# fr34kcoders/storb

Hardware: AMD Instinct MI355X
Metric: GiB/s device-resident RS encode+decode, 1 MiB chunks, 1/2/4/8 MI355X (higher is better)
Workload: dtype u8; 1 GPU; 1024 x 1 MiB chunks per GPU, RS(k=4,m=2)=zfec(4,6): encode + decode/reassemble with data shards {1,3} erased; chunks_per_gpu=1024, chunk_bytes=1048576, k=4, m_total=6, world_size=1, parallelism=chunk-partition x1

## Files before the change

include/storb_ec.h:

```cpp
#ifndef STORB_EC_H
#define STORB_EC_H

#include <stddef.h>
#include <stdint.h>

#ifdef __cplusplus
extern "C" {
#endif

#define SEC_ABI_VERSION 1

enum sec_status {
    SEC_OK = 0,
    SEC_EINVAL = -1,
    SEC_EKM = -2,
    SEC_EBLOCKLEN = -3,
    SEC_ENBLOCKS = -4,
    SEC_ESHARENUM = -5,
    SEC_EDUPSHARE = -6,
    SEC_EPADLEN = -7,
    SEC_ESIZE = -8,
    SEC_ENODEV = -9,
    SEC_EHIP = -10,
    SEC_ENOMEM = -11,
// ... 134 lines not shown
                           const int32_t *target_nums, const uint64_t *target_offs, uint8_t *out,
                           uint8_t *digests, sec_chk_result *results, uint8_t *row_bad,
                           uint8_t *column, unsigned flags);

int sec_check_locate(int k, int m, const int32_t *sharenums, int n, const uint8_t *column,
                     int32_t *culprit);

int sec_check_method(int k, int m, const int32_t *sharenums, int n, uint64_t B,
                     const uint64_t *block_avail, int64_t padlen, int *method);

int sec_ctx_check_methods(sec_ctx *ctx, int64_t *bitsliced, int64_t *direct);

int sec_repair_method(int k, int m, const int32_t *sharenums, int n, const int32_t *targets,
                      int ntargets, uint64_t B, const uint64_t *block_avail, int *method);

int sec_ctx_repair_methods(sec_ctx *ctx, int64_t *bitsliced, int64_t *direct);

typedef struct sec_msg {
    uint64_t addr;
    uint64_t len;
    uint64_t avail;
} sec_msg;

int sec_sha1_batch(sec_ctx *ctx, const sec_msg *msgs, int64_t nmsgs, uint8_t *digests, unsigned flags);

int sec_encode_digest_batch(sec_ctx *ctx, const sec_enc_chunk *chunks, int64_t nchunks,
                            const uint8_t *in, uint8_t *parity, uint8_t *digests, unsigned flags);

int sec_encode_pieces(sec_ctx *ctx, const sec_enc_chunk *chunks, int64_t nchunks, const uint8_t *in,
                      uint8_t *const *pieces, uint8_t *digests, unsigned flags);

typedef struct sec_bn_key sec_bn_key;

int sec_bn_key_create(sec_ctx *ctx, const uint8_t n_be[256], sec_bn_key **out);
void sec_bn_key_destroy(sec_bn_key *key);
int sec_bn_key_set_crt(sec_ctx *ctx, sec_bn_key *key, const uint8_t p_be[128], const uint8_t q_be[128],
                       const uint8_t cp_be[256], const uint8_t cq_be[256]);
int sec_bn_key_set_tag(sec_ctx *ctx, sec_bn_key *key, const uint8_t g_be[256], const uint8_t fdh_be[256],
                       const uint8_t d_be[256], const uint8_t *dp_be, const uint8_t *dq_be);

int sec_bn_reduce_batch(sec_ctx *ctx, const sec_bn_key *key, const sec_msg *msgs, int64_t nmsgs,
                        uint8_t *out, unsigned flags);
int sec_bn_modexp_batch(sec_ctx *ctx, const sec_bn_key *key, const uint8_t *bases,
                        const uint8_t *exps, uint32_t exp_bytes, int64_t count, uint8_t *out,
                        unsigned flags);
int sec_bn_crt_modexp_batch(sec_ctx *ctx, const sec_bn_key *key, const uint8_t *bases,
                            const uint8_t *exps_p, const uint8_t *exps_q, uint32_t exp_bytes,
                            int64_t count, uint8_t *out, unsigned flags);
int sec_apdp_gpow_batch(sec_ctx *ctx, const sec_bn_key *key, const uint8_t *exps, uint32_t exp_bytes,
                        int64_t count, uint8_t *out, unsigned flags);
int sec_bn_mulmod_batch(sec_ctx *ctx, const sec_bn_key *key, const uint8_t *a, const uint8_t *b,
                        int64_t count, uint8_t *out, unsigned flags);
int sec_apdp_tag_batch(sec_ctx *ctx, const sec_bn_key *key, const sec_msg *msgs, int64_t nmsgs,
                       uint8_t *tags, unsigned flags);

int sec_bn_crt_modexp2_batch(sec_ctx *ctx, const sec_bn_key *key, const uint8_t *a, const uint8_t *b,
                             const uint8_t *ea_p, const uint8_t *ea_q, const uint8_t *eb_p,
                             const uint8_t *eb_q, uint32_t exp_bytes, int64_t count, uint8_t *out,
                             unsigned flags);
int sec_apdp_prove_batch(sec_ctx *ctx, const sec_bn_key *key, const sec_msg *msgs, int64_t nmsgs,
                         const uint8_t *tags, const uint8_t *g_ss, const uint8_t *coefs,
                         uint8_t *tag_c, uint8_t *block, uint8_t *rho, unsigned flags);
int sec_apdp_verify_batch(sec_ctx *ctx, const sec_bn_key *key, const uint8_t *proof_tags,
                          const uint8_t *fdhs, const uint8_t *coefs, const uint8_t *ss,
                          const uint8_t e_be[256], int64_t count, uint8_t *values, int32_t *status,
                          unsigned flags);

int sec_encode_tag_batch(sec_ctx *ctx, const sec_bn_key *key, const sec_enc_chunk *chunks,
                         int64_t nchunks, const uint8_t *in, uint8_t *parity,
                         uint8_t *digests , uint8_t *tags, unsigned flags);
int sec_encode_pieces_tags(sec_ctx *ctx, const sec_bn_key *key, const sec_enc_chunk *chunks,
                           int64_t nchunks, const uint8_t *in, uint8_t *const *pieces,
                           uint8_t *digests , uint8_t *tags, unsigned flags);

int sec_malloc(sec_ctx *ctx, size_t bytes, void **dptr);
int sec_free(sec_ctx *ctx, void *dptr);
int sec_host_alloc(sec_ctx *ctx, size_t bytes, void **hptr);
int sec_host_free(sec_ctx *ctx, void *hptr);
int sec_host_register(sec_ctx *ctx, void *hptr, size_t bytes);
int sec_host_unregister(sec_ctx *ctx, void *hptr);
int sec_ctx_host_paths(sec_ctx *ctx, int64_t *zero_copy, int64_t *registered, int64_t *staged);
int sec_host_pinned_bytes(int64_t *loaned, int64_t *idle);
int sec_ctx_decode_paths(sec_ctx *ctx, int64_t *syndrome, int64_t *direct);
int sec_ctx_decode_methods(sec_ctx *ctx, int64_t *fused, int64_t *pair, int64_t *two_kernel, int64_t *direct);
int sec_memcpy(sec_ctx *ctx, void *dst, const void *src, size_t bytes, int kind);
int sec_memset(sec_ctx *ctx, void *dptr, int value, size_t bytes);
typedef struct sec_copy {
    uint64_t dst;
    uint64_t src;
    uint64_t len;
} sec_copy;
int sec_host_copy(sec_ctx *ctx, const sec_copy *jobs, int64_t njobs);

#ifdef __cplusplus
}
#endif
#endif
```

storb_amd/_build.py:

```python

from __future__ import annotations

import hashlib
import os
import subprocess

PKG = os.path.dirname(os.path.abspath(__file__))
ROOT = os.path.dirname(PKG)
CSRC = os.path.join(PKG, "csrc")
LIBDIR = os.path.join(PKG, "lib")
LIB = os.path.join(LIBDIR, "libstorbec.so")
VARIANT_DIR = os.path.join(ROOT, "build", "variants")
INCLUDE = os.path.join(ROOT, "include")
SOURCES = ["kernels.hip", "kernels_bs.hip", "bignum.hip", "api.cpp"]
HEADERS = ["kernels.hpp", "bignum.hpp", "bn_host.hpp", "bs_plan.hpp", "gf_host.hpp", "gf_const.hpp",
           "task_pool.hpp"]
ARCH = "gfx950"
HIPCC = os.environ.get("HIPCC", "/opt/rocm/bin/hipcc")


def _digest() -> str:
    h = hashlib.sha256()
    for name in SOURCES + HEADERS:
        with open(os.path.join(CSRC, name), "rb") as f:
            h.update(name.encode() + f.read())
    with open(os.path.join(INCLUDE, "storb_ec.h"), "rb") as f:
        h.update(f.read())
    h.update(ARCH.encode())
    return h.hexdigest()


def _read(path: str) -> str | None:
    try:
        with open(path) as f:
            return f.read().strip()
    except OSError:
        return None


def _includes(path: str, seen: set) -> None:
    with open(path, encoding="utf-8", errors="replace") as f:
        for line in f:
            line = line.strip()
            if line.startswith("#include \""):
                name = line.split("\"")[1]
                for d in (CSRC, INCLUDE):
                    h = os.path.join(d, name)
                    if os.path.exists(h) and h not in seen:
                        seen.add(h)
                        _includes(h, seen)


_COMPILER_ID: str | None = None


def _compiler_id() -> str:
    global _COMPILER_ID
    if _COMPILER_ID is None:
        try:
            out = subprocess.run([HIPCC, "--version"], capture_output=True, text=True, timeout=60).stdout
        except (OSError, subprocess.SubprocessError) as e:
            out = f"unavailable: {e}"
        _COMPILER_ID = HIPCC + "\n" + out
    return _COMPILER_ID


def _obj_key(src: str, flags: list) -> str:
    path = os.path.join(CSRC, src)
    deps: set = set()
    _includes(path, deps)
    h = hashlib.sha256(_compiler_id().encode() + b"\0" + " ".join(flags).encode())
    for p in [path, *sorted(deps)]:
        with open(p, "rb") as f:
            h.update(p.encode() + f.read())
    return h.hexdigest()


def variant_lib(tag: str) -> str:
    return os.path.join(VARIANT_DIR, f"libstorbec_{tag}.so")


def build(force: bool = False, verbose: bool = False, defines: dict | None = None, tag: str | None = None) -> str:
    lib = LIB if not tag else variant_lib(tag)
    os.makedirs(os.path.dirname(lib), exist_ok=True)
    defs = [f"-D{k}={v}" for k, v in sorted((defines or {}).items())]
    stamp = lib + ".stamp"
    dig = _digest() + " ".join(defs)
    if not force and os.path.exists(lib) and os.path.exists(stamp):
        with open(stamp) as f:
            if f.read().strip() == dig:
                return lib
    tmp = lib + ".tmp"
    objdir = os.path.join(os.path.dirname(lib), "obj_" + (tag or "lib"))
    os.makedirs(objdir, exist_ok=True)
    flags = [f"--offload-arch={ARCH}", "-O3", "-std=c++17", "-fPIC", "-Wall", "-Wno-unused-function",
             f"-I{INCLUDE}", *defs]
    objs, procs = [], []
    for src in SOURCES:
# ... 31 lines not shown
```

storb_amd/_lib.py:

```python

from __future__ import annotations

import ctypes
import os
import sys

import numpy as np

from ._build import LIB

SEC_OK = 0
SEC_EINVAL = -1
SEC_EKM = -2
SEC_EBLOCKLEN = -3
SEC_ENBLOCKS = -4
SEC_ESHARENUM = -5
SEC_EDUPSHARE = -6
SEC_EPADLEN = -7
SEC_ESIZE = -8
SEC_ENODEV = -9
SEC_EHIP = -10
SEC_ENOMEM = -11
SEC_ESINGULAR = -12
SEC_EMODULUS = -13
# ... 66 lines not shown
    _fields_ = [("addr", ctypes.c_uint64), ("len", ctypes.c_uint64), ("avail", ctypes.c_uint64)]


assert ENC_DTYPE.itemsize == ctypes.sizeof(sec_enc_chunk) == 40
assert MSG_DTYPE.itemsize == ctypes.sizeof(sec_msg) == 24
assert DEC_DTYPE.itemsize == ctypes.sizeof(sec_dec_chunk) == 40
assert REP_DTYPE.itemsize == ctypes.sizeof(sec_rep_chunk) == 40
assert CHK_DTYPE.itemsize == ctypes.sizeof(sec_chk_chunk) == 32
assert DCHK_DTYPE.itemsize == ctypes.sizeof(sec_dchk_chunk) == 48
assert RCHK_DTYPE.itemsize == ctypes.sizeof(sec_rchk_chunk) == 40
assert CHK_RESULT_DTYPE.itemsize == ctypes.sizeof(sec_chk_result) == 16

_vp = ctypes.c_void_p
_SIGS = {
    "sec_abi_version": (ctypes.c_int, []),
    "sec_strerror": (ctypes.c_char_p, [ctypes.c_int]),
    "sec_last_hip_error": (ctypes.c_char_p, []),
    "sec_device_count": (ctypes.c_int, [ctypes.POINTER(ctypes.c_int)]),
    "sec_ctx_create": (ctypes.c_int, [ctypes.c_int, ctypes.POINTER(_vp)]),
    "sec_ctx_destroy": (None, [_vp]),
    "sec_ctx_set_stream": (ctypes.c_int, [_vp, _vp]),
    "sec_sync": (ctypes.c_int, [_vp]),
    "sec_ctx_set_timing": (ctypes.c_int, [_vp, ctypes.c_int]),
    "sec_timing_collect": (ctypes.c_int, [_vp, ctypes.c_int, ctypes.POINTER(ctypes.c_double),
                                          ctypes.POINTER(ctypes.c_int64)]),
    "sec_ctx_set_option": (ctypes.c_int, [_vp, ctypes.c_char_p, ctypes.c_int64]),
    "sec_ctx_get_option": (ctypes.c_int, [_vp, ctypes.c_char_p, ctypes.POINTER(ctypes.c_int64)]),
    "sec_option_name": (ctypes.c_char_p, [ctypes.c_int]),
    "sec_decode_choose": (ctypes.c_int, [ctypes.c_int, ctypes.c_int, ctypes.c_int64, _vp, _vp]),
    "sec_encode_matrix": (ctypes.c_int, [ctypes.c_int, ctypes.c_int, _vp]),
    "sec_decode_matrix": (ctypes.c_int, [ctypes.c_int, ctypes.c_int, _vp, _vp, _vp]),
    "sec_encode_batch": (ctypes.c_int, [_vp, _vp, ctypes.c_int64, _vp, _vp, ctypes.c_uint]),
    "sec_decode_batch": (ctypes.c_int, [_vp, _vp, ctypes.c_int64, _vp, _vp, _vp, _vp, ctypes.c_uint]),
    "sec_decode_batch_ex": (ctypes.c_int, [_vp, _vp, ctypes.c_int64, _vp, _vp, _vp, _vp, _vp, ctypes.c_uint]),
    "sec_repair_matrix": (ctypes.c_int, [ctypes.c_int, ctypes.c_int, _vp, _vp, ctypes.c_int, _vp]),
    "sec_repair_batch": (ctypes.c_int, [_vp, _vp, ctypes.c_int64, _vp, _vp, _vp, _vp, _vp, _vp, _vp, _vp,
                                        ctypes.c_uint]),
    "sec_check_batch": (ctypes.c_int, [_vp, _vp, ctypes.c_int64, _vp, _vp, _vp, _vp, _vp, _vp, _vp, ctypes.c_uint]),
    "sec_decode_check_batch": (ctypes.c_int, [_vp, _vp, ctypes.c_int64, _vp, _vp, _vp, _vp, _vp, _vp, _vp, _vp,
                                              ctypes.c_uint]),
    "sec_repair_check_batch": (ctypes.c_int, [_vp, _vp, ctypes.c_int64, _vp, _vp, _vp, _vp, _vp, _vp, _vp, _vp, _vp, _vp,
                                              _vp, ctypes.c_uint]),
    "sec_check_locate": (ctypes.c_int, [ctypes.c_int, ctypes.c_int, _vp, ctypes.c_int, _vp,
                                        ctypes.POINTER(ctypes.c_int32)]),
    "sec_check_method": (ctypes.c_int, [ctypes.c_int, ctypes.c_int, _vp, ctypes.c_int, ctypes.c_uint64, _vp,
                                        ctypes.c_int64, ctypes.POINTER(ctypes.c_int)]),
    "sec_ctx_check_methods": (ctypes.c_int, [_vp, ctypes.POINTER(ctypes.c_int64), ctypes.POINTER(ctypes.c_int64)]),
    "sec_repair_method": (ctypes.c_int, [ctypes.c_int, ctypes.c_int, _vp, ctypes.c_int, _vp, ctypes.c_int,
                                         ctypes.c_uint64, _vp, ctypes.POINTER(ctypes.c_int)]),
    "sec_ctx_repair_methods": (ctypes.c_int, [_vp, ctypes.POINTER(ctypes.c_int64), ctypes.POINTER(ctypes.c_int64)]),
    "sec_sha1_batch": (ctypes.c_int, [_vp, _vp, ctypes.c_int64, _vp, ctypes.c_uint]),
    "sec_encode_digest_batch": (ctypes.c_int, [_vp, _vp, ctypes.c_int64, _vp, _vp, _vp, ctypes.c_uint]),
    "sec_encode_pieces": (ctypes.c_int, [_vp, _vp, ctypes.c_int64, _vp, _vp, _vp, ctypes.c_uint]),
    "sec_bn_key_create": (ctypes.c_int, [_vp, _vp, ctypes.POINTER(_vp)]),
    "sec_bn_key_destroy": (None, [_vp]),
    "sec_bn_key_set_crt": (ctypes.c_int, [_vp, _vp, _vp, _vp, _vp, _vp]),
    "sec_bn_key_set_tag": (ctypes.c_int, [_vp, _vp, _vp, _vp, _vp, _vp, _vp]),
    "sec_bn_reduce_batch": (ctypes.c_int, [_vp, _vp, _vp, ctypes.c_int64, _vp, ctypes.c_uint]),
    "sec_bn_modexp_batch": (ctypes.c_int, [_vp, _vp, _vp, _vp, ctypes.c_uint32, ctypes.c_int64, _vp,
                                           ctypes.c_uint]),
    "sec_bn_crt_modexp_batch": (ctypes.c_int, [_vp, _vp, _vp, _vp, _vp, ctypes.c_uint32, ctypes.c_int64, _vp,
                                               ctypes.c_uint]),
    "sec_apdp_gpow_batch": (ctypes.c_int, [_vp, _vp, _vp, ctypes.c_uint32, ctypes.c_int64, _vp, ctypes.c_uint]),
    "sec_bn_mulmod_batch": (ctypes.c_int, [_vp, _vp, _vp, _vp, ctypes.c_int64, _vp, ctypes.c_uint]),
    "sec_apdp_tag_batch": (ctypes.c_int, [_vp, _vp, _vp, ctypes.c_int64, _vp, ctypes.c_uint]),
    "sec_bn_crt_modexp2_batch": (ctypes.c_int, [_vp, _vp, _vp, _vp, _vp, _vp, _vp, _vp, ctypes.c_uint32,
                                                ctypes.c_int64, _vp, ctypes.c_uint]),
    "sec_apdp_prove_batch": (ctypes.c_int, [_vp, _vp, _vp, ctypes.c_int64, _vp, _vp, _vp, _vp, _vp, _vp,
                                            ctypes.c_uint]),
    "sec_apdp_verify_batch": (ctypes.c_int, [_vp, _vp, _vp, _vp, _vp, _vp, _vp, ctypes.c_int64, _vp, _vp,
                                             ctypes.c_uint]),
    "sec_encode_tag_batch": (ctypes.c_int, [_vp, _vp, _vp, ctypes.c_int64, _vp, _vp, _vp, _vp, ctypes.c_uint]),
    "sec_encode_pieces_tags": (ctypes.c_int, [_vp, _vp, _vp, ctypes.c_int64, _vp, _vp, _vp, _vp, ctypes.c_uint]),
    "sec_malloc": (ctypes.c_int, [_vp, ctypes.c_size_t, ctypes.POINTER(_vp)]),
    "sec_free": (ctypes.c_int, [_vp, _vp]),
    "sec_host_alloc": (ctypes.c_int, [_vp, ctypes.c_size_t, ctypes.POINTER(_vp)]),
    "sec_host_free": (ctypes.c_int, [_vp, _vp]),
    "sec_host_register": (ctypes.c_int, [_vp, _vp, ctypes.c_size_t]),
    "sec_host_unregister": (ctypes.c_int, [_vp, _vp]),
    "sec_ctx_host_paths": (ctypes.c_int, [_vp, ctypes.POINTER(ctypes.c_int64), ctypes.POINTER(ctypes.c_int64),
                                          ctypes.POINTER(ctypes.c_int64)]),
    "sec_host_pinned_bytes": (ctypes.c_int, [ctypes.POINTER(ctypes.c_int64), ctypes.POINTER(ctypes.c_int64)]),
    "sec_ctx_decode_paths": (ctypes.c_int, [_vp, ctypes.POINTER(ctypes.c_int64), ctypes.POINTER(ctypes.c_int64)]),
    "sec_ctx_decode_methods": (ctypes.c_int, [_vp, ctypes.POINTER(ctypes.c_int64), ctypes.POINTER(ctypes.c_int64),
                                              ctypes.POINTER(ctypes.c_int64), ctypes.POINTER(ctypes.c_int64)]),
    "sec_memcpy": (ctypes.c_int, [_vp, _vp, _vp, ctypes.c_size_t, ctypes.c_int]),
    "sec_memset": (ctypes.c_int, [_vp, _vp, ctypes.c_int, ctypes.c_size_t]),
    "sec_host_copy": (ctypes.c_int, [_vp, _vp, ctypes.c_int64]),
}
SYMBOLS = tuple(_SIGS)

_libs: dict = {}


def load(path: str | None = None) -> ctypes.CDLL:
    path = path or os.environ.get("STORB_EC_LIB", LIB)
    if path in _libs:
        return _libs[path]
    _share_torch_runtime()
    if not os.path.exists(path):
        raise ImportError(
            f"libstorbec.so not found at {path}: build it with `python -m storb_amd._build` "
            "(or __graft_entry__.build()); storb_amd has no CPU fallback")
    lib = ctypes.CDLL(path)
    for name, (res, args) in _SIGS.items():
        try:
            fn = getattr(lib, name)
        except AttributeError:
            if os.path.abspath(path) == os.path.abspath(LIB):
                raise
            continue
        fn.restype = res
        fn.argtypes = args
    if lib.sec_abi_version() != 1:
        raise ImportError("libstorbec.so ABI version mismatch")
    _libs[path] = lib
    return lib


def _share_torch_runtime() -> None:
    if "torch" in sys.modules or os.environ.get("STORB_EC_PRELOAD_TORCH", "1") == "0":
        return
    try:
        import torch
    except ImportError:
        pass


def strerror(code: int, lib: ctypes.CDLL | None = None) -> str:
    lib = lib or load()
    msg = lib.sec_strerror(code).decode()
    if code == SEC_EHIP:
        msg += ": " + lib.sec_last_hip_error().decode()
    return msg
```

storb_amd/csrc/api.cpp:

```cpp
#include <hip/hip_runtime.h>
#include <stdlib.h>
#include <string.h>
#include <sys/mman.h>

#include <algorithm>
#include <array>
#include <map>
#include <memory>
#include <mutex>
#include <set>
#include <string>
#include <thread>
#include <type_traits>
#include <utility>
#include <vector>

#include "task_pool.hpp"
#include "bignum.hpp"
#include "bn_host.hpp"
#include "bs_plan.hpp"
#include "gf_host.hpp"
#include "kernels.hpp"
#include "storb_ec.h"

namespace {

thread_local std::string g_hip_err;

int hip_fail(hipError_t e, const char *what)
{
    g_hip_err = std::string(what) + ": " + hipGetErrorString(e);
    return SEC_EHIP;
}

#define CK(x)                                   \
    do {                                        \
        hipError_t e_ = (x);                    \
        if (e_ != hipSuccess)                   \
            return hip_fail(e_, #x);            \
    } while (0)

#define RC(x)                 \
    do {                      \
        int rc_ = (x);        \
        if (rc_)              \
            return rc_;       \
    } while (0)

struct DevBuf {
    void *p = nullptr;
    size_t cap = 0;
    int ensure(size_t bytes)
    {
        if (bytes <= cap)
            return SEC_OK;
        if (p)
            CK(hipFree(p));
        p = nullptr;
        cap = 0;
        size_t want = std::max(bytes, (size_t)1 << 16);
        if (hipMalloc(&p, want) != hipSuccess) {
            p = nullptr;
            return SEC_ENOMEM;
        }
        cap = want;
        return SEC_OK;
    }
    void release()
    {
        if (p)
            (void)hipFree(p);
        p = nullptr;
        cap = 0;
    }
    template <class T> T *as(size_t off = 0) const { return reinterpret_cast<T *>((char *)p + off); }
};

constexpr size_t kPinKeep = (size_t)512 << 20;

class PinPool {
  public:
    static PinPool &get()
    {
        static PinPool *pool = new PinPool;
        return *pool;
    }
    void *take(size_t want, size_t *cap)
    {
        {
            std::lock_guard<std::mutex> lk(mu_);
            auto it = idle_.lower_bound(want);
            if (it != idle_.end()) {
                void *p = it->second;
                *cap = it->first;
                idle_bytes_ -= it->first;
                loaned_ += it->first;
                idle_.erase(it);
                return p;
            }
        }
// ... 61 lines not shown
            return SEC_ENOMEM;
        }
        cap = want;
        return SEC_OK;
    }
    void release()
    {
        if (p) {
            if (pooled)
                PinPool::get().give(p, cap);
            else
                (void)hipHostFree(p);
        }
        p = nullptr;
        cap = 0;
    }
    char *c(size_t off = 0) const { return (char *)p + off; }
};

size_t align_up(size_t v, size_t a) { return (v + a - 1) / a * a; }

enum Opt {
    O_SYN,
    O_SYN_FUSED,
    O_SYN_RATIO,
    O_BS,
    O_BS_LANES,
    O_SHA1_SPLIT,
    O_SLAB_BYTES,
    O_SLAB_BYTES_DIGEST,
    O_COPY_THREADS,
    O_REGISTER_MIN,
    O_HOST_JOIN,
    O_CHECK_BS,
    O_COUNT
};

struct OptSpec {
    const char *name;
    int64_t dflt, lo, hi;
};

constexpr OptSpec kOpts[O_COUNT] = {
    {"SEC_SYN", -1, -1, 1},
    {"SEC_SYN_FUSED", 1, 0, 1},
    {"SEC_SYN_RATIO", 900, 1, 1000000},
    {"SEC_BS", -1, -1, 1},
    {"SEC_BS_LANES", 256, 64, 256},
    {"SEC_SHA1_SPLIT", -1, -1, 1},
    {"SEC_SLAB_BYTES", (int64_t)64 << 20, (int64_t)1 << 16, (int64_t)1 << 40},
    {"SEC_SLAB_BYTES_DIGEST", (int64_t)512 << 20, (int64_t)1 << 16, (int64_t)1 << 40},
    {"SEC_COPY_THREADS", 0, 0, 256},
    {"SEC_REGISTER_MIN", (int64_t)4 << 20, 0, (int64_t)1 << 62},
    {"SEC_HOST_JOIN", 1, 0, 1},
    {"SEC_CHECK_BS", -1, -1, 1},
};

struct Options {
    int64_t v[O_COUNT];
    Options()
    {
        for (int i = 0; i < O_COUNT; ++i)
            v[i] = kOpts[i].dflt;
    }
    int64_t operator[](Opt o) const { return v[o]; }
    int lanes(Opt o) const { return (int)std::max<int64_t>(64, std::min<int64_t>(256, v[o])) / 64 * 64; }
};

int opt_index(const char *name)
{
    if (!name)
        return -1;
    for (int i = 0; i < O_COUNT; ++i)
        if (!strcmp(name, kOpts[i].name))
            return i;
    return -1;
}

struct Group {
    int rows, U, lanes, wide;
    uint32_t first, count;
    int mfma = 0;
};
using KeyedLaunches = std::vector<std::pair<int, std::pair<uint32_t, uint32_t>>>;

struct SubPlan {
    int64_t c0 = 0, c1 = 0;
    std::vector<Group> groups;
    size_t off_desc = 0, off_tiles = 0, off_tail = 0, off_soff = 0, off_srow = 0, off_mrow = 0, off_savail = 0;
    uint32_t ntail = 0;
    uint64_t in_bytes = 0, out_bytes = 0;
    size_t off_msgs = 0;
    uint32_t nmsgs = 0;
    bool sha_split = false;
    size_t off_segs = 0, off_seginfo = 0;
    uint32_t nsegs = 0, max_seg = 0;
    uint64_t dig_first = 0;
    uint64_t dig_off = 0;
    size_t off_tmsgs = 0;
    uint32_t ntmsgs = 0;
    uint64_t tag_first = 0, tag_off = 0;
    size_t off_toff = 0;
    size_t off_cpos = 0, off_echunk = 0;
    uint32_t nentries = 0;
    size_t off_cdesc = 0;
    KeyedLaunches bs_rows;
    size_t off_bs_desc = 0, off_bs_tiles = 0, off_bs_soff = 0, off_bs_avail = 0, off_bs_rmap = 0, off_bs_tmap = 0;
    uint64_t chk_rows = 0, chk_col = 0, pay_off = 0;
    std::vector<std::array<uint64_t, 3>> sha_runs;
    KeyedLaunches syn1, syn2, synf;
    size_t off_sdesc = 0, off_stiles = 0, off_ssoff = 0, off_ssavail = 0, off_vdesc = 0, off_vtiles = 0,
           off_masks = 0, off_ftiles = 0;
    uint64_t syn_bytes = 0;
    int syn_lanes = 256;
};

struct Plan {
    std::vector<uint8_t> key;
    uint64_t gen = 0;
    std::vector<SubPlan> subs;
    DevBuf meta;
    bool valid = false;
    int64_t nsyn = 0, ndirect = 0, nfused = 0;
    int64_t nrow_bs = 0, nrow_direct = 0;
    uint64_t nflags = 0;
};

struct TableCache {
    DevBuf buf;
    size_t used = 0;
    uint64_t gen = 1;
    std::map<std::string, uint32_t> index;
};

struct RowOpState {
    Plan plan;
    TableCache tabs;
    DevBuf flags;
};

struct PendingExpand {
    std::vector<uint8_t> coef;
    uint32_t dst;
};

struct Image {
    std::vector<char> bytes;
    size_t put(const void *src, size_t n)
    {
        const size_t off = align_up(bytes.size(), 256);
        bytes.resize(off + n);
        if (n)
            memcpy(bytes.data() + off, src, n);
        return off;
    }
};

int full_lanes(bool decode, bool narrow = false) { return !decode && narrow ? 64 : sec::kLanes; }

constexpr int kU = 1;

bool is_wide(int k) { return k > sec::kBatchVecs; }

using Bins = std::map<std::tuple<int, int, int, int, int>, std::vector<sec::Tile>>;

uint64_t round64(uint64_t v) { return (v + 63) / 64 * 64; }

int dec_small_kb(int k) { return k <= 4 ? 4 : 0; }

double vperm_ops(int rows, int slots)
{
// ... 82 lines not shown
#endif
#ifndef SEC_PAIR_XCD_MIN_B
#define SEC_PAIR_XCD_MIN_B (3u << 20)
#endif
constexpr int kSolveLds = 1 << 16;
constexpr int kSynWg2 = 1 << 16;

int bs_shape(const Options &o, int k, int m, uint64_t B)
{
    if (o[O_BS] == 0)
        return -1;
    if (B < 16 || B > sec::kBsMaxB)
        return -1;
    const int p = m - k;
    if (o[O_BS] != 1 && p < 8 && !(k == 10 && m == 14))
        return -1;
    return sec_bs_shape(k, m);
}

void add_bs_work(const Options &o, Bins &bins, uint32_t chunk, uint64_t B, int shape)
{
    if (sec_bs_groups(shape) > 1) {
        auto &bin = bins[{3, shape, kBsPair, 128, B >= (uint64_t)SEC_PAIR_XCD_MIN_B ? 1 : 0}];
        for (uint64_t t0 = 0; t0 < B; t0 += sec_bs_span())
            bin.push_back(sec::Tile{chunk, (uint32_t)t0, 0, 0});
        return;
    }
    const int lanes = o.lanes(O_BS_LANES);
    const uint64_t step = (uint64_t)sec_bs_span() * (lanes / 64);
    auto &bin = bins[{3, shape, 0, lanes, 0}];
    for (uint64_t t0 = 0; t0 < B; t0 += step)
        bin.push_back(sec::Tile{chunk, (uint32_t)t0, 0, 0});
}

#ifndef SEC_XCD_ORDER
#define SEC_XCD_ORDER 0
#endif


bool use_xcd_order(bool, const Group &g) { return g.mfma < 3 && SEC_XCD_ORDER == 1; }

void xcd_order(std::vector<sec::Tile> &t)
{
    const size_t n = t.size(), q = n / 8, r = n % 8;
    if (n < 16)
        return;
    std::vector<sec::Tile> o(n);
    for (size_t b = 0; b < n; ++b) {
        const size_t x = b % 8;
        o[b] = t[x * q + std::min(x, r) + b / 8];
    }
    t.swap(o);
}

void flatten(const Bins &bins, std::vector<Group> &groups, std::vector<sec::Tile> &tiles, bool decode)
{
    groups.clear();
    for (auto &kv : bins) {
        if (kv.second.empty())
            continue;
        const size_t first = tiles.size();
        tiles.insert(tiles.end(), kv.second.begin(), kv.second.end());
        groups.push_back(Group{std::get<1>(kv.first), std::get<2>(kv.first), std::get<3>(kv.first),
                               std::get<4>(kv.first), (uint32_t)first, (uint32_t)(tiles.size() - first),
                               std::get<0>(kv.first)});
        if (use_xcd_order(decode, groups.back()) || (std::get<2>(kv.first) == kBsPair && std::get<4>(kv.first))) {
            std::vector<sec::Tile> g(tiles.begin() + first, tiles.end());
            xcd_order(g);
            std::copy(g.begin(), g.end(), tiles.begin() + first);
        }
    }
}

std::vector<sec::Tile> flatten_keyed(const std::map<int, std::vector<sec::Tile>> &by_key, KeyedLaunches &launches)
{
    std::vector<sec::Tile> tiles;
    for (auto &kv : by_key) {
        launches.push_back({kv.first, {(uint32_t)tiles.size(), (uint32_t)kv.second.size()}});
        tiles.insert(tiles.end(), kv.second.begin(), kv.second.end());
    }
    return tiles;
}

template <class InBytes>
std::vector<std::pair<int64_t, int64_t>> slab_ranges(bool host, int64_t nchunks, InBytes in_bytes, size_t slab)
{
    std::vector<std::pair<int64_t, int64_t>> r;
    if (!host) {
        r.emplace_back(0, nchunks);
        return r;
    }
    int64_t c0 = 0;
    uint64_t acc = 0;
    for (int64_t i = 0; i < nchunks; ++i) {
        const uint64_t b = in_bytes(i);
        if (i > c0 && acc + b > slab) {
            r.emplace_back(c0, i);
            c0 = i;
            acc = 0;
        }
        acc += b;
    }
    if (c0 < nchunks)
        r.emplace_back(c0, nchunks);
    return r;
}

struct PlanKey {
    std::vector<uint8_t> bytes;
    PlanKey() { bytes.reserve(256); }
    void put(const void *p, size_t n)
    {
        const uint8_t *b = (const uint8_t *)p;
        bytes.insert(bytes.end(), b, b + n);
    }
    template <class T>
    void put(const T &v) { put(&v, sizeof(T)); }
};

bool plan_reusable(const Plan &plan, const TableCache &tc, const PlanKey &key)
{
    return plan.valid && plan.gen == tc.gen && plan.key == key.bytes;
}

struct Slot {
    PinBuf in, out;
    DevBuf din, dout, dsyn;
    hipStream_t s = nullptr;
    hipEvent_t done = nullptr;
    bool busy = false;
    std::vector<sec::CopyJob> scatter;
};

constexpr int kSlots = 2;

}

struct sec_ctx {
    int device = 0;
    Options opt;
    hipStream_t own = nullptr;
    hipStream_t ext = nullptr;
    bool timing = false;
    std::vector<std::pair<hipEvent_t, hipEvent_t>> pending[8];
    std::vector<hipEvent_t> ev_pool;
    hipEvent_t stop_ev = nullptr;
    PinBuf pin{nullptr, 0, false};
    hipEvent_t pin_ev = nullptr, meta_ev = nullptr;
    TableCache enc_tabs, dec_tabs;
    Plan enc_plan, dec_plan, sha_plan, bn_plan;
    RowOpState row_ops[4];
    DevBuf bn_scratch;
    DevBuf bn_part;
    DevBuf syn;
    size_t bn_part_stride = 0;
    Slot slots[kSlots];
    std::shared_ptr<sec::TaskPool> tasks;
    std::shared_ptr<sec::TaskPool> hash_tasks;
    PinBuf piece_par[2];
    int64_t zero_copy_calls = 0, registered_calls = 0, staged_calls = 0;
    int64_t syn_chunks = 0, direct_chunks = 0, fused_chunks = 0;
    int64_t chk_bs_chunks = 0, chk_direct_chunks = 0;
    int64_t rep_bs_chunks = 0, rep_direct_chunks = 0;

    hipStream_t stream() const { return ext ? ext : own; }
    hipEvent_t ev()
    {
        if (!ev_pool.empty()) {
            hipEvent_t e = ev_pool.back();
            ev_pool.pop_back();
            return e;
        }
        hipEvent_t e = nullptr;
        (void)hipEventCreate(&e);
        return e;
    }
};

namespace {

int set_dev(const sec_ctx *ctx)
{
    CK(hipSetDevice(ctx->device));
    return SEC_OK;
}

int host_threads(const sec_ctx *ctx)
{
    return ctx->opt[O_COPY_THREADS] ? (int)ctx->opt[O_COPY_THREADS] : sec::default_pool_threads();
}

sec::TaskPool &tasks(sec_ctx *ctx)
{
    if (!ctx->tasks)
        ctx->tasks = sec::shared_pool(host_threads(ctx));
    return *ctx->tasks;
}

sec::TaskPool &pool(sec_ctx *ctx) { return tasks(ctx); }

#ifndef SEC_HASH_POOL
#define SEC_HASH_POOL 1
#endif
sec::TaskPool &hash_tasks(sec_ctx *ctx)
{
    if (!SEC_HASH_POOL || ctx->opt[O_COPY_THREADS])
        return tasks(ctx);
    if (!ctx->hash_tasks)
        ctx->hash_tasks = sec::shared_pool(std::min(12, std::max(1, sec::usable_cpus() - 4)));
    return *ctx->hash_tasks;
}

#ifndef SEC_JOIN_POOL
#define SEC_JOIN_POOL 1
#endif
sec::TaskPool &join_tasks(sec_ctx *ctx) { return SEC_JOIN_POOL ? hash_tasks(ctx) : tasks(ctx); }

int slots_init(sec_ctx *ctx)
{
    for (Slot &s : ctx->slots)
        if (!s.s) {
            CK(hipStreamCreateWithFlags(&s.s, hipStreamNonBlocking));
            CK(hipEventCreateWithFlags(&s.done, hipEventDisableTiming));
        }
    return SEC_OK;
}

int slot_retire(sec_ctx *ctx, Slot &s)
{
    if (!s.busy)
        return SEC_OK;
    s.busy = false;
    CK(hipEventSynchronize(s.done));
    pool(ctx).run_copies(s.scatter);
    s.scatter.clear();
    return SEC_OK;
}

int drain_all(sec_ctx *ctx)
{
    for (Slot &s : ctx->slots) {
        RC(slot_retire(ctx, s));
        if (s.s)
            CK(hipStreamSynchronize(s.s));
    }
    CK(hipStreamSynchronize(ctx->stream()));
// ... 1 lines not shown
}

int pin_wait(sec_ctx *ctx)
{
    CK(hipEventSynchronize(ctx->pin_ev));
    return SEC_OK;
}

int table_reset(sec_ctx *ctx, TableCache &tc, size_t need_dwords)
{
    RC(drain_all(ctx));
    size_t want = std::max<size_t>(tc.buf.cap * 2, std::max<size_t>(need_dwords * 4 * 2, (size_t)1 << 20));
    tc.buf.release();
    RC(tc.buf.ensure(want));
    tc.used = 0;
    tc.index.clear();
    ++tc.gen;
    return SEC_OK;
}

void drop_pending(TableCache &tc, const std::vector<PendingExpand> &pending)
{
    if (pending.empty())
        return;
    const uint32_t first = pending.front().dst;
    for (auto it = tc.index.begin(); it != tc.index.end();)
        it = it->second >= first ? tc.index.erase(it) : std::next(it);
    tc.used = first;
}

template <class Want, class Coef>
int resolve_tables(sec_ctx *ctx, TableCache &tc, int64_t nchunks, size_t (*slack)(size_t), Want want, Coef coef,
                   std::vector<uint32_t> &tab_of, std::vector<PendingExpand> &pending)
{
    tab_of.assign((size_t)nchunks, 0);
    std::string key;
    for (int attempt = 0;; ++attempt) {
        pending.clear();
        int64_t i = 0;
        for (; i < nchunks; ++i) {
            key.clear();
            const size_t ncoef = want(i, key);
            if (!ncoef)
                continue;
            auto it = tc.index.find(key);
            if (it == tc.index.end()) {
                if ((tc.used + ncoef * sec::kTabDwords) * 4 > tc.buf.cap)
                    break;
                std::vector<uint8_t> cf;
                if (int e = coef(i, cf)) {
                    drop_pending(tc, pending);
                    return e;
                }
                it = tc.index.emplace(key, (uint32_t)tc.used).first;
                pending.push_back(PendingExpand{std::move(cf), it->second});
                tc.used += ncoef * sec::kTabDwords;
            }
            tab_of[i] = it->second;
        }
        if (i == nchunks)
            return SEC_OK;
        if (attempt == 1)
            return SEC_ENOMEM;
        size_t need = 0;
        std::set<std::string> seen;
        for (i = 0; i < nchunks; ++i) {
            key.clear();
            const size_t ncoef = want(i, key);
            if (ncoef && seen.insert(key).second)
                need += ncoef * sec::kTabDwords;
        }
        RC(table_reset(ctx, tc, slack(need)));
    }
}
size_t slack_none(size_t dwords) { return dwords; }
size_t slack_double(size_t dwords) { return dwords * 2 + ((size_t)1 << 18); }

int upload_plan_(sec_ctx *ctx, Plan &plan, Image &img, TableCache &tc, const std::vector<PendingExpand> &pending)
{
    std::vector<size_t> coef_off;
    for (const auto &pe : pending)
        coef_off.push_back(img.put(pe.coef.data(), pe.coef.size()));
    const size_t bytes = img.bytes.size();
    RC(pin_wait(ctx));
    RC(ctx->pin.ensure(bytes));
    memcpy(ctx->pin.p, img.bytes.data(), bytes);
    RC(plan.meta.ensure(bytes));
    CK(hipMemcpyAsync(plan.meta.p, ctx->pin.p, bytes, hipMemcpyHostToDevice, ctx->stream()));
    CK(hipEventRecord(ctx->pin_ev, ctx->stream()));
    for (size_t i = 0; i < pending.size(); ++i) {
        int e = sec_launch_expand(plan.meta.as<uint8_t>(coef_off[i]), (uint32_t)pending[i].coef.size(),
                                  tc.buf.as<uint32_t>() + pending[i].dst, ctx->stream());
        if (e)
            return hip_fail((hipError_t)e, "sec_expand_tables");
    }
    return SEC_OK;
}

int upload_plan(sec_ctx *ctx, Plan &plan, Image &img, TableCache &tc, const std::vector<PendingExpand> &pending)
{
    const int e = upload_plan_(ctx, plan, img, tc, pending);
    if (e)
        drop_pending(tc, pending);
    return e;
}

int timing_begin(sec_ctx *ctx, hipEvent_t *a, hipStream_t s, bool attached = true)
{
    *a = nullptr;
    if (!ctx->timing)
        return SEC_OK;
    *a = ctx->ev();
    if (attached) {
        ctx->stop_ev = ctx->ev();
        sec_launch_events(*a, ctx->stop_ev);
    } else {
        ctx->stop_ev = nullptr;
        CK(hipEventRecord(*a, s));
    }
    return SEC_OK;
}

int timing_end(sec_ctx *ctx, hipEvent_t a, int kind, hipStream_t s)
{
    if (!a)
        return SEC_OK;
    hipEvent_t b = ctx->stop_ev;
    ctx->stop_ev = nullptr;
    if (b) {
        if (sec_launch_events(nullptr, nullptr) == 0) {
            CK(hipEventRecord(a, s));
            CK(hipEventRecord(b, s));
        }
    } else {
        b = ctx->ev();
        CK(hipEventRecord(b, s));
    }
    ctx->pending[kind].emplace_back(a, b);
    return SEC_OK;
}

bool sha1_split(const Options &o, const std::vector<sec::MsgDesc> &md)
{
    if (o[O_SHA1_SPLIT] >= 0)
        return o[O_SHA1_SPLIT] == 1;
    if (md.empty())
        return false;
    uint64_t blocks = 0;
    for (const sec::MsgDesc &m : md)
        blocks += m.len / 64;
    return md.size() <= ((size_t)16 << 10) && blocks / md.size() >= 256;
}

int check_sharenums(int k, int m, const int32_t *s)
{
    bool seen[256] = {false};
    for (int i = 0; i < k; ++i) {
        if (s[i] < 0 || s[i] >= m)
            return SEC_ESHARENUM;
        if (seen[s[i]])
            return SEC_EDUPSHARE;
        seen[s[i]] = true;
    }
    return SEC_OK;
}

int check_blocks(int k, int m, const int32_t *held, int n, const int32_t *targets, int nt, bool in_turn)
{
    if (nt < 0 || !held || (nt > 0 && !targets) || (!in_turn && n < 0))
        return SEC_EINVAL;
    if (k < 1 || m < k || m > 256)
        return SEC_EKM;
// ... 95 lines not shown

int build_encode_plan(sec_ctx *ctx, const sec_enc_chunk *chunks, int64_t nchunks, bool host, int digest, bool tag)
{
    Plan &plan = ctx->enc_plan;
    TableCache &tc = ctx->enc_tabs;
    std::vector<PendingExpand> pending;
    std::vector<uint32_t> tab_of;
    auto want = [&](int64_t i, std::string &key) {
        const int k = chunks[i].k, m = chunks[i].m;
        if (m > k)
            key = std::to_string(k) + "/" + std::to_string(m);
        return (size_t)k * (m - k);
    };
    auto coef = [&](int64_t i, std::vector<uint8_t> &cf) {
        const int k = chunks[i].k, p = chunks[i].m - k;
        const std::vector<uint8_t> enc = sec::encode_matrix(k, chunks[i].m);
        cf.resize((size_t)k * p);
        for (int j = 0; j < k; ++j)
            for (int r = 0; r < p; ++r)
                cf[(size_t)j * p + r] = enc[(size_t)(k + r) * k + j];
        return (int)SEC_OK;
    };
    RC(resolve_tables(ctx, tc, nchunks, slack_none, want, coef, tab_of, pending));

    const auto ranges = slab_ranges(host, nchunks, [&](int64_t i) { return chunks[i].n; },
                                    (size_t)ctx->opt[digest || tag ? O_SLAB_BYTES_DIGEST : O_SLAB_BYTES]);
    Image img;
    plan.subs.clear();
    bool narrow = true;
    for (int64_t i = 0; i < nchunks && narrow; ++i)
        if (chunks[i].m > chunks[i].k && enc_B(chunks[i]) < ((uint64_t)64 << 10))
            narrow = false;
    uint64_t dig = 0, tags = 0;
    for (auto [c0, c1] : ranges) {
        SubPlan sp;
        sp.c0 = c0;
        sp.c1 = c1;
        sp.dig_first = dig;
        sp.tag_first = tags;
        std::vector<sec::EncDesc> descs((size_t)(c1 - c0));
        Bins bins;
        std::vector<sec::TailItem> tail;
        std::vector<sec::MsgDesc> msgs, tmsgs;
        const bool all = digest == 1 || (tag && !digest);
        for (int64_t i = c0; i < c1; ++i) {
            const sec_enc_chunk &c = chunks[i];
            const uint64_t B = enc_B(c);
            const int p = c.m - c.k;
            const int64_t valid = (int64_t)c.n - (int64_t)(c.k - 1) * (int64_t)B;
            sec::EncDesc &d = descs[i - c0];
            d.in_off = host ? sp.in_bytes : c.in_off;
            d.par_off = host ? sp.out_bytes : c.parity_off;
            d.par_stride = host ? B : c.parity_stride;
            d.B = (uint32_t)B;
            d.k = (uint32_t)c.k;
            d.p = (uint32_t)p;
            d.tab = tab_of[i];
            d.valid = (uint32_t)std::max<int64_t>(0, std::min<int64_t>(valid, (int64_t)B));
            d.pad = 0;
            if (digest || tag) {
                for (int j = 0; j < c.k && (all || tag); ++j) {
                    const int64_t av = (int64_t)c.n - (int64_t)j * (int64_t)B;
                    (all ? msgs : tmsgs)
                        .push_back(sec::MsgDesc{d.in_off + (uint64_t)j * B, B,
                                                (uint64_t)std::max<int64_t>(0, std::min<int64_t>(av, (int64_t)B)), 0,
                                                0});
                }
                for (int r = 0; r < p; ++r) {
                    msgs.push_back(sec::MsgDesc{d.par_off + (uint64_t)r * d.par_stride, B, B, 1, 0});
                    if (tag && !all)
                        tmsgs.push_back(msgs.back());
                }
                dig += (uint64_t)(digest == 1 ? c.m : digest ? p : 0);
                tags += (uint64_t)(tag ? c.m : 0);
            }
            sp.in_bytes += c.n;
            sp.out_bytes += (uint64_t)p * B;
            const int bs = p > 0 ? bs_shape(ctx->opt, c.k, c.m, B) : -1;
            if (bs >= 0)
                add_bs_work(ctx->opt, bins, (uint32_t)(i - c0), B, bs);
            else if (p > 0)
                add_work(bins, tail, (uint32_t)(i - c0), B, valid, p, c.k, false, narrow);
        }
        std::vector<sec::Tile> tiles;
        flatten(bins, sp.groups, tiles, false);
        sp.ntail = (uint32_t)tail.size();
        sp.dig_off = sp.out_bytes;
        if (host && digest)
            sp.out_bytes += (uint64_t)msgs.size() * 20;
        sp.tag_off = sp.out_bytes;
        sp.off_desc = img.put(descs.data(), descs.size() * sizeof(sec::EncDesc));
        sp.off_tiles = img.put(tiles.data(), tiles.size() * sizeof(sec::Tile));
        sp.off_tail = img.put(tail.data(), tail.size() * sizeof(sec::TailItem));
        put_msgs(ctx->opt, sp, img, msgs);
        if (tag) {
            const std::vector<sec::MsgDesc> &tm = all ? msgs : tmsgs;
            sp.ntmsgs = (uint32_t)tm.size();
            sp.off_tmsgs = all ? sp.off_msgs : img.put(tm.data(), tm.size() * sizeof(sec::MsgDesc));
            put_segs(sp, img, tm, kSegBytes);
            if (host)
                sp.out_bytes += (uint64_t)tm.size() * 256;
            if (!digest)
                sp.nmsgs = 0;
        }
        plan.subs.push_back(std::move(sp));
    }
    RC(upload_plan(ctx, plan, img, tc, pending));
    plan.gen = tc.gen;
    return SEC_OK;
}

int launch_encode_sub(sec_ctx *ctx, const Plan &plan, const SubPlan &sp, const uint8_t *in, uint8_t *par,
                      uint8_t *digests, hipStream_t s)
{
    const sec::EncDesc *dd = plan.meta.as<sec::EncDesc>(sp.off_desc);
    const sec::Tile *dt = plan.meta.as<sec::Tile>(sp.off_tiles);
    const uint32_t *tabs = ctx->enc_tabs.buf.as<uint32_t>();
    for (const Group &g : sp.groups) {
        int e = g.mfma == 3 ? sec_launch_encode_bs(g.rows, g.U == kBsPair ? -2 : g.U, g.lanes, in, par, dd,
                                                   dt + g.first, g.count, s)
                            : sec_launch_encode(g.rows, g.U, g.wide, g.lanes, in, par, dd, dt + g.first, g.count, tabs, s);
        if (e)
            return hip_fail((hipError_t)e, g.mfma == 3 ? "sec_encode_bs_kernel" : "sec_encode_kernel");
    }
    if (sp.ntail) {
        int e = sec_launch_encode_tail(in, par, dd, plan.meta.as<sec::TailItem>(sp.off_tail), sp.ntail, tabs, s);
        if (e)
            return hip_fail((hipError_t)e, "sec_encode_tail");
    }
    if (sp.nmsgs) {
        int e = sec_launch_sha1(in, par, plan.meta.as<sec::MsgDesc>(sp.off_msgs), sp.nmsgs, digests, s, sp.sha_split);
        if (e)
            return hip_fail((hipError_t)e, "sec_sha1_kernel");
    }
    return SEC_OK;
}

int launch_encode_tags(sec_ctx *ctx, const Plan &plan, const SubPlan &sp, const sec_bn_key *key, const uint8_t *in,
                       const uint8_t *par, uint8_t *tags, bool host, hipStream_t s)
{
    hipEvent_t t0;
    RC(timing_begin(ctx, &t0, s, false));
    int e = sec_launch_apdp_tag(key->dk.as<sec::TagKey>(), key->table.as<uint32_t>(), key->rpow.as<uint32_t>(), in, par,
                                plan.meta.as<sec::MsgDesc>(sp.off_tmsgs), sp.ntmsgs,
                                plan.meta.as<sec::SegDesc>(sp.off_segs), sp.nsegs,
                                plan.meta.as<sec::SegInfo>(sp.off_seginfo),
                                bn_part(ctx, (size_t)(&sp - plan.subs.data()), host), tags, s);
    if (e)
        return hip_fail((hipError_t)e, "sec_apdp_tag");
    return timing_end(ctx, t0, 3, s);
}

struct SlotLayout {
    std::vector<int> perm, idx;
    std::vector<uint64_t> first;
};

template <class Chunk>
SlotLayout slot_layout(const Chunk *chunks, int64_t nchunks, const int32_t *sharenums)
{
    SlotLayout L;
    L.first.resize((size_t)nchunks);
    std::vector<int> idx, perm;
    for (int64_t i = 0; i < nchunks; ++i) {
        const Chunk &c = chunks[i];
        idx.assign(sharenums + c.slot0, sharenums + c.slot0 + c.k);
        sec::normalise_slots(c.k, idx, perm);
        L.first[i] = L.perm.size();
        L.perm.insert(L.perm.end(), perm.begin(), perm.end());
        L.idx.insert(L.idx.end(), idx.begin(), idx.end());
    }
    return L;
}

template <class Chunk>
uint64_t slot_avail(const Chunk &c, const uint64_t *block_avail, int j)
{
    return block_avail ? std::min<uint64_t>(block_avail[c.slot0 + j], c.B) : c.B;
}

bool check_bs_rule(const Options &o, int shape, uint64_t B, bool copies)
{
    if (o[O_CHECK_BS] >= 0)
        return o[O_CHECK_BS] == 1;
    switch (shape) {
    case 0: return B <= (8u << 10);
    case 2: return !copies && B >= (64u << 10);
    case 3:
    case 4: return B >= (4u << 10);
    default: return false;
    }
}

bool repair_bs_rule(const Options &o, int shape, uint64_t B, int nt, int nr)
{
    if (o[O_CHECK_BS] >= 0)
        return o[O_CHECK_BS] == 1;
    const int rows = nt + nr;
    switch (shape) {
    case 0: return B == 6554 && rows == 4 && nt <= 2;
// ... 185 lines not shown
                    sp.syn_bytes += (uint64_t)e * sec::syn_stride(c.B);
                uint64_t lost = 0;
                for (int s = 0; s < k; ++s)
                    if (idx[s] >= k)
                        lost |= 1ull << s;
                const std::string key = slots_key(k, c.m, idx);
                auto mk = mask_of.find(key);
                if (mk == mask_of.end()) {
                    std::vector<int> S, Lost;
                    for (int r = 0; r < p; ++r)
                        if ((sd.pmask >> r) & 1)
                            S.push_back(r);
                    for (int s = 0; s < k; ++s)
                        if ((lost >> s) & 1)
                            Lost.push_back(s);
                    std::vector<uint8_t> w, z;
                    sec::cauchy_scales(k, S, Lost, w, z);
                    const std::pair<uint32_t, uint32_t> at{(uint32_t)masks.size(), (uint32_t)(masks.size() + e)};
                    for (uint8_t v : w)
                        masks.push_back(sec::scale_mask(v));
                    for (uint8_t v : z)
                        masks.push_back(sec::scale_mask(v));
                    mk = mask_of.emplace(key, at).first;
                }
                sd.wq0 = mk->second.first;
                sd.zq0 = mk->second.second;
                sd.flags = recover ? 2u : 0u;
                const uint32_t si = (uint32_t)sdescs.size();
                sdescs.push_back(sd);
                const uint64_t step = (uint64_t)sec_bs_span() * (syn_lanes / 64);
                if (method == kSynFused) {
                    auto &ft = ftiles[sh];
                    for (uint64_t t = 0; t < c.B; t += step)
                        ft.push_back(sec::Tile{si, (uint32_t)t, (uint32_t)(gs[0] * NR), copies ? 1u : 0u});
                    continue;
                }
                if (gs.size() == 2 && sec_syn_pair(sh)) {
                    auto &st2 = stiles[kSynWg2 + sh];
                    for (uint64_t t = 0; t < c.B; t += sec_bs_span())
                        st2.push_back(sec::Tile{si, (uint32_t)t, 0u, copies ? 1u : 0u});
                } else {
                    sec::add_group_run_tiles(stiles[sh], si, c.B, step, gs, NR, copies);
                }
                sec::SolveDesc vd{};
                vd.out_off = d.out_off;
                vd.syn_off = sd.syn_off;
                vd.lost = lost;
                vd.pmask = sd.pmask;
                vd.B = (uint32_t)c.B;
                vd.last = last;
                vd.zq0 = mk->second.second;
                vd.recover = recover ? 1u : 0u;
                const uint32_t vi = (uint32_t)vdescs.size();
                vdescs.push_back(vd);
                if (sec_solve_lds(sh)) {
                    auto &vt = vtiles[kSolveLds + sh * 64 + ((e + 7) / 8) * 8];
                    for (uint64_t t = 0; t < c.B; t += sec_bs_span())
                        vt.push_back(sec::Tile{vi, (uint32_t)t, 0u, 0u});
                    continue;
                }
                const int NR2 = sec_solve_rows(sh);
                sec::add_group_run_tiles(vtiles[sh], vi, c.B, step, sec::touched_groups(lost, k, NR2), NR2, false);
            } else if (nout > 0 && !(nocopy && e_of[i] == 0)) {
                add_work(bins, tail, (uint32_t)(i - c0), c.B, valid, (int)e_of[i], c.k, true, false,
                         recover || nocopy ? dec_small_kb(c.k) : 0);
            }
        }
        if (SEC_DEC_XCD_BIG) {
            auto big = [&](const std::vector<sec::Tile> &t, auto B_of) {
                for (const sec::Tile &x : t)
                    if (B_of(x) >= (uint64_t)SEC_PAIR_XCD_MIN_B)
                        return true;
                return false;
            };
            auto sB = [&](const sec::Tile &x) { return (uint64_t)sdescs[x.chunk].B; };
            auto vB = [&](const sec::Tile &x) { return (uint64_t)vdescs[x.chunk].B; };
            for (auto &kv : stiles)
                if (kv.first >= kSynWg2 && big(kv.second, sB))
                    xcd_order(kv.second);
            for (auto &kv : vtiles)
                if (kv.first >= kSolveLds && big(kv.second, vB))
                    xcd_order(kv.second);
        }
        std::vector<sec::Tile> tiles;
        flatten(bins, sp.groups, tiles, true);
        const std::vector<sec::Tile> stl = flatten_keyed(stiles, sp.syn1), vtl = flatten_keyed(vtiles, sp.syn2),
                                     ftl = flatten_keyed(ftiles, sp.synf);
        sp.off_ftiles = img.put(ftl.data(), ftl.size() * sizeof(sec::Tile));
        sp.off_sdesc = img.put(sdescs.data(), sdescs.size() * sizeof(sec::SynDesc));
        sp.off_stiles = img.put(stl.data(), stl.size() * sizeof(sec::Tile));
        sp.off_ssoff = img.put(ssoff.data(), ssoff.size() * 8);
        sp.off_ssavail = img.put(ssavail.data(), ssavail.size() * 4);
        sp.off_vdesc = img.put(vdescs.data(), vdescs.size() * sizeof(sec::SolveDesc));
        sp.off_vtiles = img.put(vtl.data(), vtl.size() * sizeof(sec::Tile));
        sp.off_masks = img.put(masks.data(), masks.size() * 8);
        sp.ntail = (uint32_t)tail.size();
        sp.off_desc = img.put(descs.data(), descs.size() * sizeof(sec::DecDesc));
        sp.off_tiles = img.put(tiles.data(), tiles.size() * sizeof(sec::Tile));
        sp.off_tail = img.put(tail.data(), tail.size() * sizeof(sec::TailItem));
        soff.resize(soff.size() + sec::kBatchVecs, 0);
        sp.off_soff = img.put(soff.data(), soff.size() * 8);
        sp.off_srow = img.put(srow.data(), srow.size() * 4);
        sp.off_mrow = img.put(mrow.data(), mrow.size() * 4);
        sp.off_savail = img.put(savail.data(), savail.size() * 4);
        plan.subs.push_back(std::move(sp));
    }
    RC(upload_plan(ctx, plan, img, tc, pending));
    plan.gen = tc.gen;
    return SEC_OK;
}

int launch_decode_sub(sec_ctx *ctx, const Plan &plan, const SubPlan &sp, const uint8_t *blocks, uint8_t *out,
                      hipStream_t s, uint8_t *syn = nullptr)
{
    const sec::DecDesc *dd = plan.meta.as<sec::DecDesc>(sp.off_desc);
    const sec::Tile *dt = plan.meta.as<sec::Tile>(sp.off_tiles);
    const uint32_t *tabs = ctx->dec_tabs.buf.as<uint32_t>();
    const sec::DecSlots sl{plan.meta.as<uint64_t>(sp.off_soff), plan.meta.as<uint32_t>(sp.off_srow),
                           plan.meta.as<uint32_t>(sp.off_mrow), plan.meta.as<uint32_t>(sp.off_savail)};
    for (const Group &g : sp.groups) {
        int e = sec_launch_rows(g.rows, g.U, g.wide, g.lanes, blocks, out, dd, dt + g.first, g.count, tabs, sl, s,
                                g.mfma);
        if (e)
            return hip_fail((hipError_t)e, "sec_decode_kernel");
    }
    if (sp.ntail) {
        int e = sec_launch_rows_tail(blocks, out, dd, plan.meta.as<sec::TailItem>(sp.off_tail), sp.ntail, tabs, sl, s);
        if (e)
            return hip_fail((hipError_t)e, "sec_decode_tail");
    }
    if (sp.syn1.empty() && sp.synf.empty())
        return SEC_OK;
    if (!syn && !sp.syn1.empty())
        return SEC_EINVAL;
    const uint64_t *masks = plan.meta.as<uint64_t>(sp.off_masks);
    const sec::SynDesc *sd = plan.meta.as<sec::SynDesc>(sp.off_sdesc);
    const sec::Tile *st = plan.meta.as<sec::Tile>(sp.off_stiles);
    const sec::SynSlots ss{plan.meta.as<uint64_t>(sp.off_ssoff), plan.meta.as<uint32_t>(sp.off_ssavail), masks};
    const int lanes = sp.syn_lanes;
    const sec::Tile *ft = plan.meta.as<sec::Tile>(sp.off_ftiles);
    for (const auto &g : sp.synf) {
        int e = sec_launch_decode_bs(g.first, lanes, blocks, out, sd, ft + g.second.first, g.second.second, ss, s);
        if (e)
            return hip_fail((hipError_t)e, "sec_decode_bs_kernel");
    }
    for (const auto &g : sp.syn1) {
        const bool wg2 = g.first >= kSynWg2;
        int e = wg2 ? sec_launch_syndrome_bs_pair(g.first - kSynWg2, blocks, out, syn, sd, st + g.second.first,
                                                  g.second.second, ss, s)
                    : sec_launch_syndrome_bs(g.first, lanes, blocks, out, syn, sd, st + g.second.first,
                                             g.second.second, ss, s);
        if (e)
            return hip_fail((hipError_t)e, wg2 ? "sec_syndrome_bs_pair_kernel" : "sec_syndrome_bs_kernel");
    }
    const sec::SolveDesc *vd = plan.meta.as<sec::SolveDesc>(sp.off_vdesc);
    const sec::Tile *vt = plan.meta.as<sec::Tile>(sp.off_vtiles);
    for (const auto &g : sp.syn2) {
        const bool staged = g.first >= kSolveLds;
        int e = staged ? sec_launch_solve_bs_lds((g.first - kSolveLds) / 64, (g.first - kSolveLds) % 64, syn, out, vd,
                                                 vt + g.second.first, g.second.second, masks, s)
                       : sec_launch_solve_bs(g.first, lanes, syn, out, vd, vt + g.second.first, g.second.second, masks, s);
        if (e)
            return hip_fail((hipError_t)e, staged ? "sec_solve_bs_lds_kernel" : "sec_solve_bs_kernel");
    }
    return SEC_OK;
}


struct RowChunk {
    uint64_t B, slot0, tgt0, out_off, padlen;
    int k, m;
    int n;
    int nt;
};

struct RowArgs {
    const int32_t *sharenums;
    const uint64_t *block_offs, *block_avail;
    const uint8_t *blocks;
    const int32_t *target_nums;
    const uint64_t *target_offs;
    uint8_t *out, *digests;
    sec_chk_result *results;
    uint8_t *row_bad, *column;
    unsigned flags;
};

struct RowInfo {
    uint32_t B, k, ns, nr, tab, slot0, tgt0, flag0, valid;
    uint64_t out_off, nout;
};

sec::ChkDesc chk_desc(const RowInfo &r, uint32_t res, uint32_t cslot0)
{
    return {r.B, r.k, r.nr, r.tab, r.slot0, r.flag0, r.valid, res, cslot0, 0};
}

int check_held(const RowChunk &c, const RowArgs &a, const int32_t *targets = nullptr)
{
    return check_blocks(c.k, c.m, a.sharenums + c.slot0, c.n, targets, c.nt, false);
}

// ... 2325 lines not shown
    if (B >= (1ull << 31))
        return SEC_ESIZE;
    *method = sec::repair_bs_shape(sec_bs_shape(k, m), k, sharenums, n, ntargets, B, block_avail) >= 0 ? 1 : 0;
    return SEC_OK;
}

int sec_check_locate(int k, int m, const int32_t *sharenums, int n, const uint8_t *column, int32_t *culprit)
{
    RC(check_blocks(k, m, sharenums, k, sharenums ? sharenums + k : nullptr, n - k, true));
    if (!column || !culprit)
        return SEC_EINVAL;
    int who = -2;
    if (!sec::check_locate(k, m, std::vector<int>(sharenums, sharenums + n), column, &who))
        return SEC_ESINGULAR;
    *culprit = who;
    return SEC_OK;
}

int sec_malloc(sec_ctx *ctx, size_t bytes, void **dptr)
{
    if (!ctx || !dptr)
        return SEC_EINVAL;
    RC(set_dev(ctx));
    if (hipMalloc(dptr, bytes ? bytes : 1) != hipSuccess)
        return SEC_ENOMEM;
    return SEC_OK;
}

int sec_free(sec_ctx *ctx, void *dptr)
{
    if (!ctx)
        return SEC_EINVAL;
    RC(set_dev(ctx));
    CK(hipFree(dptr));
    return SEC_OK;
}

int sec_host_alloc(sec_ctx *ctx, size_t bytes, void **hptr)
{
    if (!ctx || !hptr)
        return SEC_EINVAL;
    RC(set_dev(ctx));
    if (hipHostMalloc(hptr, bytes ? bytes : 1, hipHostMallocDefault) != hipSuccess)
        return SEC_ENOMEM;
    return SEC_OK;
}

int sec_host_free(sec_ctx *ctx, void *hptr)
{
    (void)ctx;
    CK(hipHostFree(hptr));
    return SEC_OK;
}

int sec_host_register(sec_ctx *ctx, void *hptr, size_t bytes)
{
    if (!ctx || !hptr || !bytes)
        return SEC_EINVAL;
    RC(set_dev(ctx));
    CK(hipHostRegister(hptr, bytes, hipHostRegisterDefault));
    return SEC_OK;
}

int sec_host_unregister(sec_ctx *ctx, void *hptr)
{
    (void)ctx;
    if (!hptr)
        return SEC_EINVAL;
    CK(hipHostUnregister(hptr));
    return SEC_OK;
}

int sec_ctx_decode_paths(sec_ctx *ctx, int64_t *syndrome, int64_t *direct)
{
    if (!ctx)
        return SEC_EINVAL;
    if (syndrome)
        *syndrome = ctx->syn_chunks;
    if (direct)
        *direct = ctx->direct_chunks;
    return SEC_OK;
}

int sec_ctx_decode_methods(sec_ctx *ctx, int64_t *fused, int64_t *pair, int64_t *two_kernel, int64_t *direct)
{
    if (!ctx)
        return SEC_EINVAL;
    if (fused)
        *fused = ctx->fused_chunks;
    if (pair)
        *pair = 0;
    if (two_kernel)
        *two_kernel = ctx->syn_chunks - ctx->fused_chunks;
    if (direct)
        *direct = ctx->direct_chunks;
    return SEC_OK;
}

int sec_ctx_check_methods(sec_ctx *ctx, int64_t *bitsliced, int64_t *direct)
{
    if (!ctx)
        return SEC_EINVAL;
    if (bitsliced)
        *bitsliced = ctx->chk_bs_chunks;
    if (direct)
        *direct = ctx->chk_direct_chunks;
    return SEC_OK;
}

int sec_ctx_repair_methods(sec_ctx *ctx, int64_t *bitsliced, int64_t *direct)
{
    if (!ctx)
        return SEC_EINVAL;
    if (bitsliced)
        *bitsliced = ctx->rep_bs_chunks;
    if (direct)
        *direct = ctx->rep_direct_chunks;
    return SEC_OK;
}

int sec_host_pinned_bytes(int64_t *loaned, int64_t *idle)
{
    PinPool::get().stats(loaned, idle);
    return SEC_OK;
}

int sec_ctx_host_paths(sec_ctx *ctx, int64_t *zero_copy, int64_t *registered, int64_t *staged)
{
    if (!ctx || !zero_copy || !registered || !staged)
        return SEC_EINVAL;
    *zero_copy = ctx->zero_copy_calls;
    *registered = ctx->registered_calls;
    *staged = ctx->staged_calls;
    return SEC_OK;
}

int sec_memcpy(sec_ctx *ctx, void *dst, const void *src, size_t bytes, int kind)
{
    if (!ctx || (bytes && (!dst || !src)) || kind < 0 || kind > 2)
        return SEC_EINVAL;
    RC(set_dev(ctx));
    static const hipMemcpyKind kinds[3] = {hipMemcpyHostToDevice, hipMemcpyDeviceToHost, hipMemcpyDeviceToDevice};
    if (bytes) {
        CK(hipMemcpyAsync(dst, src, bytes, kinds[kind], ctx->stream()));
        CK(hipStreamSynchronize(ctx->stream()));
    }
    return SEC_OK;
}

int sec_host_copy(sec_ctx *ctx, const sec_copy *jobs, int64_t njobs)
{
    if (!ctx || njobs < 0 || (njobs > 0 && !jobs))
        return SEC_EINVAL;
    std::vector<sec::CopyJob> cj;
    cj.reserve((size_t)njobs);
    for (int64_t i = 0; i < njobs; ++i) {
        if (!jobs[i].len)
            continue;
        if (!jobs[i].dst)
            return SEC_EINVAL;
        cj.push_back(sec::CopyJob{(void *)(uintptr_t)jobs[i].dst, (const void *)(uintptr_t)jobs[i].src,
                                  (size_t)jobs[i].len});
    }
    join_tasks(ctx).run_copies(cj);
    return SEC_OK;
}
// ... 15 lines not shown
```

storb_amd/csrc/kernels.hip:

```cpp
#include <hip/hip_ext.h>
#include <hip/hip_runtime.h>

#include <type_traits>

#include "kernels.hpp"

using u8 = uint8_t;
using u32 = uint32_t;
using u64 = uint64_t;
typedef u32 u32x4 __attribute__((ext_vector_type(4)));
typedef u32x4 u32x4_u __attribute__((aligned(1)));

namespace {

struct GfTables {
    u8 exp[512];
    u8 log[256];
};

constexpr GfTables make_gf()
{
    GfTables t{};
    u32 v = 1;
    for (int e = 0; e < 255; ++e) {
        t.exp[e] = (u8)v;
        t.exp[e + 255] = (u8)v;
        t.log[v] = (u8)e;
        v <<= 1;
        if (v & 0x100)
            v ^= 0x11D;
    }
    t.exp[510] = t.exp[0];
    t.exp[511] = t.exp[1];
    t.log[0] = 255;
    return t;
}

__constant__ GfTables c_gf = make_gf();

__global__ __launch_bounds__(256) void sec_expand_tables(const u8 *__restrict__ coef, u32 ncoef,
                                                         u32 *__restrict__ tabs)
{
    __shared__ u8 s_exp[512];
    __shared__ u8 s_log[256];
    for (u32 i = threadIdx.x; i < 512; i += blockDim.x)
        s_exp[i] = c_gf.exp[i];
    for (u32 i = threadIdx.x; i < 256; i += blockDim.x)
        s_log[i] = c_gf.log[i];
    __syncthreads();
    const u32 i = blockIdx.x * blockDim.x + threadIdx.x;
    if (i >= ncoef)
        return;
    const u32 c = coef[i];
    const u32 lc = s_log[c];
    auto mul = [&](u32 v) -> u32 { return (c && v) ? (u32)s_exp[lc + s_log[v]] : 0u; };
    auto pack = [&](u32 a, u32 b, u32 cc, u32 d) { return mul(a) | mul(b) << 8 | mul(cc) << 16 | mul(d) << 24; };
    u32 *o = tabs + (u64)i * sec::kTabDwords;
    o[0] = pack(0, 1, 2, 3);
    o[1] = pack(4, 5, 6, 7);
    o[2] = pack(0 << 3, 1 << 3, 2 << 3, 3 << 3);
    o[3] = pack(4 << 3, 5 << 3, 6 << 3, 7 << 3);
    o[4] = pack(0 << 6, 1 << 6, 2 << 6, 3 << 6);
}

__device__ __forceinline__ u32 xor3(u32 a, u32 b, u32 c)
{
    u32 r;
    asm("v_bitop3_b32 %0, %1, %2, %3 bitop3:0x96" : "=v"(r) : "v"(a), "v"(b), "v"(c));
    return r;
}
__device__ __forceinline__ u32 bfi(u32 b, u32 c, u32 d)
{
    u32 r;
    asm("v_bfi_b32 %0, %1, %2, %3" : "=v"(r) : "v"(b), "v"(c), "v"(d));
    return r;
}
__device__ __forceinline__ u32 maj(u32 a, u32 b, u32 c)
{
    u32 r;
    asm("v_bitop3_b32 %0, %1, %2, %3 bitop3:0xe8" : "=v"(r) : "v"(a), "v"(b), "v"(c));
    return r;
}

template <int U>
struct Sel {
    u32 s0[U][4], s1[U][4], s2[U][4];
    __device__ __forceinline__ explicit Sel(const u32x4 (&x)[U])
// ... 134 lines not shown
#endif
#ifndef SEC_DEC_BATCH
#define SEC_DEC_BATCH sec::kBatchVecs
#endif
#ifndef SEC_ENC_BATCH
#define SEC_ENC_BATCH sec::kBatchVecs
#endif
#ifndef SEC_WIDE_BATCH
#define SEC_WIDE_BATCH 8
#endif
template <int U, bool W, bool DEC>
constexpr int batch_blocks()
{
    constexpr int v = (W && SEC_WIDE_BATCH > 0) ? SEC_WIDE_BATCH : (DEC ? SEC_DEC_BATCH : SEC_ENC_BATCH);
    return v / U > 0 ? v / U : 1;
}

__device__ __forceinline__ u32x4 load16(const u8 *p)
{
#if SEC_NT_LOAD
    return __builtin_nontemporal_load(reinterpret_cast<const u32x4_u *>(p));
#else
    return *reinterpret_cast<const u32x4_u *>(p);
#endif
}
template <int POL>
__device__ __forceinline__ void store16(u8 *p, u32x4 v)
{
    if constexpr (POL == 0)
        *reinterpret_cast<u32x4_u *>(p) = v;
    else if constexpr (POL == 1)
        __builtin_nontemporal_store(v, reinterpret_cast<u32x4_u *>(p));
    else if constexpr (POL == 2)
        asm volatile("global_store_dwordx4 %0, %1, off nt sc1\n\ts_nop 1" ::"v"(p), "v"(v) : "memory");
    else
        asm volatile("global_store_dwordx4 %0, %1, off sc0 sc1\n\ts_nop 1" ::"v"(p), "v"(v) : "memory");
}

__device__ __forceinline__ u32 gf_mul_byte(const u32 *__restrict__ t, u32 x)
{
    return (__builtin_amdgcn_perm(t[1], t[0], x & 7u) ^ __builtin_amdgcn_perm(t[3], t[2], (x >> 3) & 7u) ^
            __builtin_amdgcn_perm(t[4], t[4], x >> 6)) & 0xFFu;
}

template <int U>
__device__ __forceinline__ void tile_pos(u32 (&pos)[U], u32 t, u32 valid)
{
    const u32 step = blockDim.x * sec::kLaneBytes;
#pragma unroll
    for (int u = 0; u < U; ++u)
        pos[u] = min(t + u * step, valid - sec::kLaneBytes);
}

template <int R, int N>
__device__ __forceinline__ void gf_mac_bytes(u32 (&acc)[N], const u32 *__restrict__ tab, u32 row0, u32 x)
{
#pragma unroll
    for (int r = 0; r < R; ++r)
        acc[r] ^= gf_mul_byte(tab + (row0 + r) * sec::kTabDwords, x);
}

template <int R, int U, bool W>
__device__ __forceinline__ void encode_main(const u8 *__restrict__ in, u8 *__restrict__ par, const sec::EncDesc &d,
                                            const sec::Tile &tl, const u32 *__restrict__ tabs, u32 t);
template <int R>
__device__ __forceinline__ void encode_ragged(const u8 *__restrict__ in, u8 *__restrict__ par, const sec::EncDesc &d,
                                           const sec::Tile &tl, const u32 *__restrict__ tabs);

template <int R, int U, bool W>
__global__ __launch_bounds__(sec::max_lanes(R, U)) void sec_encode_kernel(const u8 *__restrict__ in, u8 *__restrict__ par,
                                                         const sec::EncDesc *__restrict__ descs,
                                                         const sec::Tile *__restrict__ tiles,
                                                         const u32 *__restrict__ tabs)
{
    const sec::Tile tl = tiles[blockIdx.x];
    const sec::EncDesc d = descs[tl.chunk];
    const u32 t = tl.t0 + threadIdx.x * sec::kLaneBytes;
    if (t < d.valid)
        encode_main<R, U, W>(in, par, d, tl, tabs, t);
    if (tl.ntail)
        encode_ragged<R>(in, par, d, tl, tabs);
}

template <int R, int U, bool W>
__device__ __forceinline__ void encode_main(const u8 *__restrict__ in, u8 *__restrict__ par, const sec::EncDesc &d,
                                            const sec::Tile &tl, const u32 *__restrict__ tabs, u32 t)
{
    const u32 B = d.B, k = d.k;
    u32 pos[U];
    tile_pos(pos, t, d.valid);
    const u8 *row = in + d.in_off;
    u8 *dst = par + d.par_off + (u64)tl.r0 * d.par_stride;
    const u32 *tj = tabs + d.tab + tl.r0 * sec::kTabDwords;
    const u32 tstep = d.p * sec::kTabDwords;

    u32x4 acc[R][U];
#pragma unroll
    for (int r = 0; r < R; ++r)
#pragma unroll
        for (int u = 0; u < U; ++u)
            acc[r][u] = u32x4{0u, 0u, 0u, 0u};

    constexpr int KB = batch_blocks<U, W, false>();
    auto batch = [&](u32 j0) {
        constexpr bool LT = lds_tab<R, false>();
        const u32x2 *vt = wave_tabs<KB, R, LT>(tj, tstep, j0, k);
        u32x4 xs[KB][U];
#pragma unroll
        for (int c = 0; c < KB; ++c)
            if (j0 + c < k) {
#pragma unroll
                for (int u = 0; u < U; ++u)
                    xs[c][u] = load16(row + (u64)(j0 + c) * B + pos[u]);
            }
        if constexpr (kPairRows<R, W>()) {
#pragma unroll
            for (int c = 0; c < KB; c += 2) {
                if (c + 1 < KB && j0 + c + 1 < k)
                    gf_mac2<R, U, LT>(acc, xs[c], tj + (j0 + c) * tstep, vt + c * R, xs[c + 1],
                                  tj + (j0 + c + 1) * tstep, vt + (c + 1) * R);
                else if (j0 + c < k)
                    gf_mac<R, U, LT>(acc, xs[c], tj + (j0 + c) * tstep, vt + c * R);
            }
        } else {
#pragma unroll
            for (int c = 0; c < KB; ++c)
                if (j0 + c < k)
                    gf_mac<R, U, LT>(acc, xs[c], tj + (j0 + c) * tstep, vt + c * R);
        }
    };
    if constexpr (W) {
#pragma unroll 1
        for (u32 j0 = 0; j0 < k; j0 += KB)
            batch(j0);
    } else {
        batch(0);
    }
#pragma unroll
    for (int r = 0; r < R; ++r)
#pragma unroll
        for (int u = 0; u < U; ++u)
            store16<SEC_ENC_ST>(dst + (u64)r * d.par_stride + pos[u], acc[r][u]);
}

__device__ __forceinline__ u32 ragged_lane0(u32 valid, u32 t0)
{
    const u32 used = min(blockDim.x, (valid - t0 + sec::kLaneBytes - 1) / sec::kLaneBytes);
    return (threadIdx.x + blockDim.x - used) % blockDim.x;
}

constexpr u32 kBatch = 16;

template <class Slots>
__device__ __forceinline__ void load_slot_bytes(u32 (&x)[kBatch], const u8 *__restrict__ blocks, const Slots &sl,
                                                u32 slot0, u32 c0, u32 k, u32 tp)
{
#pragma unroll
    for (u32 q = 0; q < kBatch; ++q)
        x[q] = (c0 + q < k && tp < sl.avail[slot0 + c0 + q]) ? (u32)blocks[sl.off[slot0 + c0 + q] + tp] : 0u;
}

template <int R>
__device__ __forceinline__ void encode_ragged(const u8 *__restrict__ in, u8 *__restrict__ par, const sec::EncDesc &d,
                                              const sec::Tile &tl, const u32 *__restrict__ tabs)
{
    const u8 *src = in + d.in_off;
    const u32 nblk = d.k - 1;
    for (u32 i = ragged_lane0(d.valid, tl.t0); i < tl.ntail; i += blockDim.x) {
        const u32 tp = d.valid + i;
        u32 acc[R];
#pragma unroll
        for (int r = 0; r < R; ++r)
            acc[r] = 0;
        for (u32 j0 = 0; j0 < nblk; j0 += kBatch) {
            u32 x[kBatch];
#pragma unroll
            for (u32 q = 0; q < kBatch; ++q)
                x[q] = j0 + q < nblk ? (u32)src[(u64)(j0 + q) * d.B + tp] : 0u;
#pragma unroll
            for (u32 q = 0; q < kBatch; ++q)
                if (j0 + q < nblk) {
                    const u32 *tj = tabs + d.tab + ((j0 + q) * d.p + tl.r0) * sec::kTabDwords;
#pragma unroll
                    for (int r = 0; r < R; ++r)
                        acc[r] ^= gf_mul_byte(tj + r * sec::kTabDwords, x[q]);
                }
        }
#pragma unroll
        for (int r = 0; r < R; ++r)
            par[d.par_off + (u64)(tl.r0 + r) * d.par_stride + tp] = (u8)acc[r];
    }
}

__global__ __launch_bounds__(256) void sec_encode_tail(const u8 *__restrict__ in, u8 *__restrict__ par,
                                                       const sec::EncDesc *__restrict__ descs,
                                                       const sec::TailItem *__restrict__ items, u32 nitems,
                                                       const u32 *__restrict__ tabs)
{
    const u32 i = blockIdx.x * blockDim.x + threadIdx.x;
    if (i >= nitems)
        return;
    const sec::TailItem it = items[i];
    const sec::EncDesc d = descs[it.chunk];
    const u8 *src = in + d.in_off + it.t;
    for (u32 r = 0; r < d.p; ++r) {
        u32 acc = 0;
        for (u32 j = 0; j < d.k; ++j) {
            const u32 x = (j + 1 < d.k || it.t < d.valid) ? (u32)src[(u64)j * d.B] : 0u;
            acc ^= gf_mul_byte(tabs + d.tab + (j * d.p + r) * sec::kTabDwords, x);
        }
        par[d.par_off + (u64)r * d.par_stride + it.t] = (u8)acc;
    }
}

template <int R, int U, bool W, int KBX>
__device__ __forceinline__ void decode_main(const u8 *__restrict__ blocks, u8 *__restrict__ out,
                                            const sec::DecDesc &d, const sec::Tile &tl, u32 t,
                                            const u32 *__restrict__ tabs, const sec::DecSlots sl);
template <int R>
__device__ __forceinline__ void decode_ragged(const u8 *__restrict__ blocks, u8 *__restrict__ out, const sec::DecDesc &d,
                                           const sec::Tile &tl, const u32 *__restrict__ tabs,
                                           const sec::DecSlots sl);

template <int R, int U, bool W, int KBX>
__global__ __launch_bounds__(sec::max_lanes(R, U)) void sec_decode_kernel(const u8 *__restrict__ blocks, u8 *__restrict__ out,
                                                         const sec::DecDesc *__restrict__ descs,
                                                         const sec::Tile *__restrict__ tiles,
                                                         const u32 *__restrict__ tabs,
                                                         const sec::DecSlots sl)
{
    const sec::Tile tl = tiles[blockIdx.x];
    const sec::DecDesc d = descs[tl.chunk];
    const u32 t = tl.t0 + threadIdx.x * sec::kLaneBytes;
    if (t < d.valid)
        decode_main<R, U, W, KBX>(blocks, out, d, tl, t, tabs, sl);
    if (tl.ntail)
        decode_ragged<R>(blocks, out, d, tl, tabs, sl);
}

template <int R>
__device__ __forceinline__ void decode_ragged(const u8 *__restrict__ blocks, u8 *__restrict__ out, const sec::DecDesc &d,
                                              const sec::Tile &tl, const u32 *__restrict__ tabs,
                                              const sec::DecSlots sl)
{
    for (u32 i = ragged_lane0(d.valid, tl.t0); i < tl.ntail; i += blockDim.x) {
        const u32 tp = d.valid + i;
        u8 *dst = out + d.out_off + tp;
        u32 acc[R > 0 ? R : 1];
#pragma unroll
        for (int r = 0; r < R; ++r)
            acc[r] = 0;
        for (u32 c0 = 0; c0 < d.k; c0 += kBatch) {
            u32 x[kBatch];
            load_slot_bytes(x, blocks, sl, d.slot0, c0, d.k, tp);
#pragma unroll
            for (u32 q = 0; q < kBatch; ++q)
                if (c0 + q < d.k) {
                    const u32 c = c0 + q;
                    const u32 orow = sl.row[d.slot0 + c];
                    if (tl.r0 == 0 && orow != 0xFFFFFFFFu && (u64)orow * d.B + tp < d.n)
                        dst[(u64)orow * d.B] = (u8)x[q];
                    gf_mac_bytes<R>(acc, tabs + d.tab, c * d.e + tl.r0, x[q]);
                }
        }
#pragma unroll
        for (int r = 0; r < R; ++r) {
            const u32 orow = sl.miss[d.slot0 + tl.r0 + r];
            if ((u64)orow * d.B + tp < d.n)
                dst[(u64)orow * d.B] = (u8)acc[r];
        }
    }
}

template <int R, int U, bool W, int KBX>
__device__ __forceinline__ void decode_main(const u8 *__restrict__ blocks, u8 *__restrict__ out,
                                            const sec::DecDesc &d, const sec::Tile &tl, u32 t,
                                            const u32 *__restrict__ tabs,
                                                         const sec::DecSlots sl)
{
    const u32 B = d.B, k = d.k;
    u32 pos[U];
    tile_pos(pos, t, d.valid);
    u8 *dst = out + d.out_off;
    const bool copies = tl.r0 == 0;
    const u32 *tj = tabs + d.tab + tl.r0 * sec::kTabDwords;
    const u32 tstep = d.e * sec::kTabDwords;

    u32x4 acc[R > 0 ? R : 1][U];
#pragma unroll
    for (int r = 0; r < (R > 0 ? R : 1); ++r)
#pragma unroll
        for (int u = 0; u < U; ++u)
            acc[r][u] = u32x4{0u, 0u, 0u, 0u};

    constexpr int KB = KBX > 0 ? KBX : batch_blocks<U, W, true>();
    auto batch = [&](u32 c0) {
        constexpr bool LT = lds_tab<R, true>();
        const u32x2 *vt = wave_tabs<KB, R, LT>(tj, tstep, c0, k);
        u64 so[KB];
        const u64 *sop = sl.off + d.slot0 + c0;
#pragma unroll
        for (int c = 0; c < KB; ++c)
            so[c] = sop[c];
        u32x4 xs[KB][U];
#pragma unroll
        for (int c = 0; c < KB; ++c)
            if (c0 + c < k) {
                const u8 *s = blocks + so[c];
#pragma unroll
                for (int u = 0; u < U; ++u)
                    xs[c][u] = load16(s + pos[u]);
            }
        if constexpr (R > 0 && kPairRows<R, W>()) {
#pragma unroll
            for (int c = 0; c < KB; c += 2) {
                if (c + 1 < KB && c0 + c + 1 < k)
                    gf_mac2<R, U, LT>(acc, xs[c], tj + (c0 + c) * tstep, vt + c * R, xs[c + 1],
                                      tj + (c0 + c + 1) * tstep, vt + (c + 1) * R);
                else if (c0 + c < k)
                    gf_mac<R, U, LT>(acc, xs[c], tj + (c0 + c) * tstep, vt + c * R);
            }
        } else if constexpr (R > 0) {
#pragma unroll
            for (int c = 0; c < KB; ++c)
                if (c0 + c < k)
                    gf_mac<R, U, LT>(acc, xs[c], tj + (c0 + c) * tstep, vt + c * R);
        }
#pragma unroll
        for (int c = 0; c < KB; ++c)
            if (c0 + c < k) {
                const u32 orow = sl.row[d.slot0 + c0 + c];
                if (copies && orow != 0xFFFFFFFFu) {
                    u8 *o = dst + (u64)orow * B;
#pragma unroll
                    for (int u = 0; u < U; ++u)
                        store16<SEC_DEC_ST>(o + pos[u], xs[c][u]);
                }
            }
    };
    if constexpr (W) {
#pragma unroll 1
        for (u32 c0 = 0; c0 < k; c0 += KB)
            batch(c0);
    } else {
        batch(0);
    }
    if constexpr (R > 0) {
#pragma unroll
        for (int r = 0; r < R; ++r) {
            u8 *o = dst + (u64)sl.miss[d.slot0 + tl.r0 + r] * B;
#pragma unroll
            for (int u = 0; u < U; ++u)
                store16<SEC_DEC_ST>(o + pos[u], acc[r][u]);
        }
    }
}

__global__ __launch_bounds__(256) void sec_decode_tail(const u8 *__restrict__ blocks, u8 *__restrict__ out,
                                                       const sec::DecDesc *__restrict__ descs,
                                                       const sec::TailItem *__restrict__ items, u32 nitems,
                                                       const u32 *__restrict__ tabs,
                                                       const sec::DecSlots sl)
{
    const u32 i = blockIdx.x * blockDim.x + threadIdx.x;
    if (i >= nitems)
        return;
    const sec::TailItem it = items[i];
    const sec::DecDesc d = descs[it.chunk];
    u8 *dst = out + d.out_off + it.t;
    auto slot_byte = [&](u32 c) -> u32 {
        return it.t < sl.avail[d.slot0 + c] ? (u32)blocks[sl.off[d.slot0 + c] + it.t] : 0u;
    };
    for (u32 c = 0; c < d.k; ++c) {
        const u32 orow = sl.row[d.slot0 + c];
        if (orow != 0xFFFFFFFFu && (u64)orow * d.B + it.t < d.n)
            dst[(u64)orow * d.B] = (u8)slot_byte(c);
    }
    for (u32 r = 0; r < d.e; ++r) {
        const u32 orow = sl.miss[d.slot0 + r];
        if ((u64)orow * d.B + it.t >= d.n)
            continue;
        u32 acc = 0;
        for (u32 c = 0; c < d.k; ++c)
// ... 1134 lines not shown
    return with_rows<1>(rows, [&](auto r) {
        constexpr int R = decltype(r)::value;
        return launch_shm(sec_encode_kernel<R, U, W>, dim3(nt), dim3(lanes),
                          lds_tab_bytes<batch_blocks<U, W, false>(), R, false>(lanes), s, in, par, d, t, tabs);
    });
}

template <class Desc>
struct RowKernels;
#define SEC_ROW_KERNELS(Desc, R0, OUT, TILE, TAIL)                                 \
    template <>                                                                    \
    struct RowKernels<sec::Desc> {                                                 \
        static constexpr int kRows0 = R0;                                          \
        static constexpr bool kOut = OUT;                                          \
        template <int R, bool W, int KBX>                                          \
        static constexpr auto tile() { return TILE<R, 1, W, KBX>; }                \
        static constexpr auto tail() { return TAIL; }                              \
    }
SEC_ROW_KERNELS(DecDesc, 0, true, sec_decode_kernel, sec_decode_tail);
SEC_ROW_KERNELS(RepDesc, 1, true, sec_repair_kernel, sec_repair_tail);
SEC_ROW_KERNELS(ChkDesc, 1, false, sec_check_kernel, sec_check_tail);
SEC_ROW_KERNELS(DChkDesc, 0, true, sec_decode_check_kernel, sec_decode_check_tail);
SEC_ROW_KERNELS(RChkDesc, 1, true, sec_repair_check_kernel, sec_repair_check_tail);
#undef SEC_ROW_KERNELS

template <bool W, int KBX, class Desc, class Slots>
hipError_t dispatch_rows(int rows, const u8 *b, u8 *o, const Desc *d, const sec::Tile *t, u32 nt, const u32 *tabs,
                         Slots sl, u32 lanes, hipStream_t s)
{
    using K = RowKernels<Desc>;
    return with_rows<K::kRows0>(rows, [&](auto r) {
        constexpr int R = decltype(r)::value;
        constexpr int KB = KBX > 0 ? KBX : batch_blocks<1, W, true>();
        const u32 shm = lds_tab_bytes<KB, R, true>(lanes);
        if constexpr (K::kOut)
            return launch_shm(K::template tile<R, W, KBX>(), dim3(nt), dim3(lanes), shm, s, b, o, d, t, tabs, sl);
        else
            return launch_shm(K::template tile<R, W, KBX>(), dim3(nt), dim3(lanes), shm, s, b, d, t, tabs, sl);
    });
}

}

void sec_next_launch_events(void **start, void **stop)
{
    *start = t_start;
    t_start = nullptr;
    *stop = t_stop;
    ++t_launched;
}

int sec_launch_events(void *start, void *stop)
{
    const int n = t_launched;
    t_start = (hipEvent_t)start;
    t_stop = (hipEvent_t)stop;
    t_launched = 0;
    return n;
}

int sec_launch_expand(const uint8_t *coef, uint32_t ncoef, uint32_t *tabs, void *stream)
{
    if (ncoef == 0)
        return hipSuccess;
    return launch(sec_expand_tables, dim3((ncoef + 255) / 256), dim3(256), (hipStream_t)stream, coef, ncoef, tabs);
}

int sec_launch_encode(int rows, int U, int wide, int lanes, const uint8_t *in, uint8_t *par,
                      const sec::EncDesc *descs, const sec::Tile *tiles, uint32_t ntiles, const uint32_t *tabs,
                      void *stream)
{
    if (ntiles == 0)
        return hipSuccess;
    if (lanes < 64 || lanes % 64 || lanes > sec::max_lanes(rows, U) || (wide && U != 1))
        return hipErrorInvalidValue;
    hipStream_t s = (hipStream_t)stream;
    if (wide)
        return dispatch_enc<1, true>(rows, in, par, descs, tiles, ntiles, tabs, (u32)lanes, s);
    if (U != 1)
        return hipErrorInvalidValue;
    return dispatch_enc<1, false>(rows, in, par, descs, tiles, ntiles, tabs, (u32)lanes, s);
}

int sec_launch_encode_tail(const uint8_t *in, uint8_t *par, const sec::EncDesc *descs, const sec::TailItem *items,
                           uint32_t nitems, const uint32_t *tabs, void *stream)
{
    if (nitems == 0)
        return hipSuccess;
    return launch(sec_encode_tail, dim3((nitems + 255) / 256), dim3(256), (hipStream_t)stream, in, par, descs, items,
                  nitems, tabs);
}

template <class Desc, class Slots>
int sec_launch_rows(int rows, int U, int wide, int lanes, const uint8_t *blocks, uint8_t *out, const Desc *descs,
                    const sec::Tile *tiles, uint32_t ntiles, const uint32_t *tabs, Slots sl, void *stream, int kb)
{
    if (ntiles == 0)
        return hipSuccess;
    if (rows < RowKernels<Desc>::kRows0 || U != 1 || lanes < 64 || lanes % 64 || lanes > sec::max_lanes(rows, U))
        return hipErrorInvalidValue;
    hipStream_t s = (hipStream_t)stream;
    const u32 L = (u32)lanes;
    if (kb) {
        if (wide || kb != 4)
            return hipErrorInvalidValue;
        return dispatch_rows<false, 4>(rows, blocks, out, descs, tiles, ntiles, tabs, sl, L, s);
    }
    if (wide)
        return dispatch_rows<true, 0>(rows, blocks, out, descs, tiles, ntiles, tabs, sl, L, s);
    return dispatch_rows<false, 0>(rows, blocks, out, descs, tiles, ntiles, tabs, sl, L, s);
}

template <class Desc, class Slots>
int sec_launch_rows_tail(const uint8_t *blocks, uint8_t *out, const Desc *descs, const sec::TailItem *items,
                         uint32_t nitems, const uint32_t *tabs, Slots sl, void *stream)
{
    if (nitems == 0)
        return hipSuccess;
    using K = RowKernels<Desc>;
    const dim3 grid((nitems + 255) / 256), block(256);
    if constexpr (K::kOut)
        return launch(K::tail(), grid, block, (hipStream_t)stream, blocks, out, descs, items, nitems, tabs, sl);
    else
        return launch(K::tail(), grid, block, (hipStream_t)stream, blocks, descs, items, nitems, tabs, sl);
}

#define SEC_ROW_LAUNCHERS(Desc, Slots)                                                                              \
    template int sec_launch_rows(int, int, int, int, const uint8_t *, uint8_t *, const sec::Desc *,                 \
                                 const sec::Tile *, uint32_t, const uint32_t *, sec::Slots, void *, int);           \
    template int sec_launch_rows_tail(const uint8_t *, uint8_t *, const sec::Desc *, const sec::TailItem *,         \
                                      uint32_t, const uint32_t *, sec::Slots, void *)
SEC_ROW_LAUNCHERS(DecDesc, DecSlots);

int sec_launch_sha1(const uint8_t *base0, const uint8_t *base1, const sec::MsgDesc *msgs, uint32_t nmsgs,
                    uint8_t *digests, void *stream, int split)
{
    if (nmsgs == 0)
        return hipSuccess;
    if (split)
        return launch(sec_sha1_split_kernel, dim3((nmsgs + 63) / 64), dim3(128), (hipStream_t)stream, base0, base1,
                      msgs, nmsgs, digests);
    if (SEC_SHA1_PF)
        return launch(sec_sha1_kernel<true>, dim3((nmsgs + 63) / 64), dim3(64), (hipStream_t)stream, base0, base1, msgs,
                      nmsgs, digests);
    return launch(sec_sha1_kernel<false>, dim3((nmsgs + 63) / 64), dim3(64), (hipStream_t)stream, base0, base1, msgs,
                  nmsgs, digests);
}

SEC_ROW_LAUNCHERS(RepDesc, RepSlots);
SEC_ROW_LAUNCHERS(ChkDesc, ChkSlots);
SEC_ROW_LAUNCHERS(DChkDesc, DChkSlots);
SEC_ROW_LAUNCHERS(RChkDesc, RChkSlots);
#undef SEC_ROW_LAUNCHERS

int sec_launch_check_final(const uint8_t *blocks, const sec::ChkDesc *descs, uint32_t nentries, sec::ChkSlots sl,
                           sec::ChkResult *results, uint8_t *row_bad, uint8_t *column, void *stream)
{
    if (nentries == 0)
        return hipSuccess;
    return launch(sec_check_final, dim3((nentries + 255) / 256), dim3(256), (hipStream_t)stream, blocks, descs,
                  nentries, sl, results, row_bad, column);
}
```

storb_amd/csrc/kernels.hpp:

```cpp
#pragma once
#include <stdint.h>

namespace sec {

constexpr int kLanes = 256;
constexpr int kLaneBytes = 16;
constexpr int kStepBytes = kLanes * kLaneBytes;
constexpr int kMaxRows = 8;
constexpr int kTabDwords = 5;
constexpr int kBatchVecs = 16;
#ifndef SEC_LB_WIDE_ROWS
#define SEC_LB_WIDE_ROWS 1024
#endif
constexpr int max_lanes(int rows, int U) { return U != 1 ? kLanes : (rows > 4 ? SEC_LB_WIDE_ROWS : 1024); }

struct EncDesc {
    uint64_t in_off;
    uint64_t par_off;
    uint64_t par_stride;
    uint32_t B;
    uint32_t k;
    uint32_t p;
    uint32_t tab;
    uint32_t valid;
// ... 148 lines not shown
    const uint64_t *off;
    const uint32_t *avail;
    const uint32_t *rmap;
    uint32_t *flags;
};

struct RbsDesc {
    uint64_t pmask;
    uint64_t tmask;
    uint32_t B;
    uint32_t slot0;
    uint32_t flag0;
    uint32_t rmap0;
};

struct RbsSlots {
    const uint64_t *off;
    const uint32_t *avail;
    const uint32_t *rmap;
    const uint32_t *tmap;
    const uint64_t *tgt_off;
    uint32_t *flags;
};

constexpr uint64_t kSynSpan = 2048;
constexpr uint64_t syn_stride(uint64_t B) { return (B + kSynSpan - 1) / kSynSpan * kSynSpan; }

struct Tile {
    uint32_t chunk;
    uint32_t t0;
    uint32_t r0;
    uint32_t ntail;
};

struct TailItem {
    uint32_t chunk;
    uint32_t t;
};

struct MsgDesc {
    uint64_t off;
    uint64_t len;
    uint64_t avail;
    uint32_t base;
    uint32_t pad;
};

}

extern "C++" {
int sec_launch_events(void *start, void *stop);
void sec_next_launch_events(void **start, void **stop);
int sec_launch_expand(const uint8_t *coef, uint32_t ncoef, uint32_t *tabs, void *stream);
int sec_launch_encode(int rows, int U, int wide, int lanes, const uint8_t *in, uint8_t *par,
                      const sec::EncDesc *descs, const sec::Tile *tiles, uint32_t ntiles, const uint32_t *tabs,
                      void *stream);
int sec_bs_shape(int k, int m, int rows = 0);
int sec_bs_groups(int shape);
int sec_bs_rows(int shape);
uint32_t sec_bs_span();
int sec_launch_encode_bs(int shape, int group, int lanes, const uint8_t *in, uint8_t *par, const sec::EncDesc *descs,
                         const sec::Tile *t, uint32_t ntiles, void *stream);
int sec_syn_shape(int k, int m);
int sec_launch_syndrome_bs(int shape, int lanes, const uint8_t *blocks, uint8_t *out, uint8_t *syn,
                           const sec::SynDesc *descs, const sec::Tile *t, uint32_t ntiles, sec::SynSlots sl,
                           void *stream);
int sec_launch_syndrome_bs_pair(int shape, const uint8_t *blocks, uint8_t *out, uint8_t *syn, const sec::SynDesc *descs,
                                const sec::Tile *t, uint32_t ntiles, sec::SynSlots sl, void *stream);
int sec_launch_decode_bs(int shape, int lanes, const uint8_t *blocks, uint8_t *out, const sec::SynDesc *descs,
                         const sec::Tile *t, uint32_t ntiles, sec::SynSlots sl, void *stream);
int sec_launch_check_bs(int shape, int lanes, const uint8_t *blocks, uint8_t *out, const sec::CbsDesc *descs,
                        const sec::Tile *t, uint32_t ntiles, sec::CbsSlots sl, void *stream);
int sec_launch_repair_bs(int shape, int lanes, const uint8_t *blocks, uint8_t *out, const sec::RbsDesc *descs,
                         const sec::Tile *t, uint32_t ntiles, sec::RbsSlots sl, void *stream);
int sec_syn_pair(int shape);
int sec_solve_rows(int shape);
int sec_solve_lds(int shape);
int sec_launch_solve_bs_lds(int shape, int slots, const uint8_t *syn, uint8_t *out, const sec::SolveDesc *descs,
                            const sec::Tile *t, uint32_t ntiles, const uint64_t *masks, void *stream);
int sec_launch_solve_bs(int shape, int lanes, const uint8_t *syn, uint8_t *out, const sec::SolveDesc *descs,
                        const sec::Tile *t, uint32_t ntiles, const uint64_t *masks, void *stream);
int sec_launch_encode_tail(const uint8_t *in, uint8_t *par, const sec::EncDesc *descs, const sec::TailItem *items,
                           uint32_t nitems, const uint32_t *tabs, void *stream);
int sec_launch_sha1(const uint8_t *base0, const uint8_t *base1, const sec::MsgDesc *msgs, uint32_t nmsgs,
                    uint8_t *digests, void *stream, int split = 0);
template <class Desc, class Slots>
int sec_launch_rows(int rows, int U, int wide, int lanes, const uint8_t *blocks, uint8_t *out, const Desc *descs,
                    const sec::Tile *tiles, uint32_t ntiles, const uint32_t *tabs, Slots slots, void *stream,
                    int kb = 0);
template <class Desc, class Slots>
int sec_launch_rows_tail(const uint8_t *blocks, uint8_t *out, const Desc *descs, const sec::TailItem *items,
                         uint32_t nitems, const uint32_t *tabs, Slots slots, void *stream);
int sec_launch_check_final(const uint8_t *blocks, const sec::ChkDesc *descs, uint32_t nentries, sec::ChkSlots slots,
                           sec::ChkResult *results, uint8_t *row_bad, uint8_t *column, void *stream);
}
```

storb_amd/csrc/kernels_bs.hip:

```cpp
#include <hip/hip_ext.h>
#if defined(__HIP_DEVICE_COMPILE__) && !defined(__gfx950__)
#error "libstorbec is written for gfx950 (MI355X) only: 16-byte global_load_lds, v_bitop3, 64+ KiB LDS"
#endif
#include <hip/hip_runtime.h>

#include <type_traits>
#include <utility>

#include "gf_const.hpp"
#include "kernels.hpp"

namespace {

using u8 = uint8_t;
using u32 = uint32_t;
using u64 = uint64_t;
typedef u32 u32x4 __attribute__((ext_vector_type(4)));
typedef u32x4 u32x4_u __attribute__((aligned(1)));

constexpr u32 kSpan = 2048;

constexpr u32 plane_mask(u32 c, int i)
{
    u32 m = 0;
    for (int s = 0; s < 8; ++s)
        if ((gfc::gmul(c, 1u << s) >> i) & 1u)
            m |= 1u << s;
    return m;
}
static_assert(plane_mask(1, 3) == 8 && plane_mask(2, 0) == 0x80 && plane_mask(2, 1) == 0x01, "plane masks");

__device__ __forceinline__ u32 xor3(u32 a, u32 b, u32 c)
{
    u32 r;
    asm("v_bitop3_b32 %0, %1, %2, %3 bitop3:0x96" : "=v"(r) : "v"(a), "v"(b), "v"(c));
    return r;
}

__device__ __forceinline__ u32 bfi(u32 m, u32 x, u32 y)
{
    u32 r;
    asm("v_bfi_b32 %0, %1, %2, %3" : "=v"(r) : "s"(m), "v"(x), "v"(y));
    return r;
}

template <int S, u32 MK>
__device__ __forceinline__ void swap_bits(u32 &a, u32 &b)
{
    constexpr u32 HI = MK << S;
    const u32 na = bfi(HI, b << S, a);
    const u32 nb = bfi(MK, a >> S, b);
    a = na;
    b = nb;
}

__device__ __forceinline__ void transpose8(u32 (&x)[8])
{
    swap_bits<4, 0x0F0F0F0Fu>(x[0], x[4]);
    swap_bits<4, 0x0F0F0F0Fu>(x[1], x[5]);
    swap_bits<4, 0x0F0F0F0Fu>(x[2], x[6]);
    swap_bits<4, 0x0F0F0F0Fu>(x[3], x[7]);
    swap_bits<2, 0x33333333u>(x[0], x[2]);
    swap_bits<2, 0x33333333u>(x[1], x[3]);
    swap_bits<2, 0x33333333u>(x[4], x[6]);
    swap_bits<2, 0x33333333u>(x[5], x[7]);
    swap_bits<1, 0x55555555u>(x[0], x[1]);
    swap_bits<1, 0x55555555u>(x[2], x[3]);
    swap_bits<1, 0x55555555u>(x[4], x[5]);
    swap_bits<1, 0x55555555u>(x[6], x[7]);
}

template <bool NT>
__device__ __forceinline__ u32x4 ld16(const u8 *p)
{
    if constexpr (NT)
        return __builtin_nontemporal_load(reinterpret_cast<const u32x4_u *>(p));
    else
        return *reinterpret_cast<const u32x4_u *>(p);
}

template <bool NT>
__device__ __forceinline__ u32x4 ld16_avail(const u8 *base, u32 off, u32 avail)
{
    if (off + 16 <= avail)
        return ld16<NT>(base + off);
    u32 w[4] = {0, 0, 0, 0};
#pragma unroll
    for (int b = 0; b < 16; ++b)
        if (off + b < avail)
            w[b >> 2] |= (u32)base[off + b] << (8 * (b & 3));
    return u32x4{w[0], w[1], w[2], w[3]};
}
// ... 73 lines not shown
    x[6] = b.z;
    x[7] = b.w;
}

template <int K, int M, int R0, int NR, int D, bool NT, int J>
__device__ __forceinline__ void one_block(u32 (&acc)[NR * 8], u32 (&ring)[D][8], const u8 *src, u64 B, u32 pa,
                                          u32 pb, u32 valid)
{
    u32 x[8];
#pragma unroll
    for (int i = 0; i < 8; ++i)
        x[i] = ring[J % D][i];
    if constexpr (J + D < K)
        load_block<NT>(ring[J % D], src + (u64)(J + D) * B, pa, pb, valid, J + D == K - 1);
    transpose8(x);
    u32 lo[16], hi[16];
    subsets(x[0], x[1], x[2], x[3], lo);
    subsets(x[4], x[5], x[6], x[7], hi);
    block_rows<K, M, R0, J, J == 0>(std::make_integer_sequence<int, NR * 8>{}, acc, lo, hi);
}

template <int K, int M, int R0, int NR, int D, bool NT, int... Js>
__device__ __forceinline__ void all_blocks(std::integer_sequence<int, Js...>, u32 (&acc)[NR * 8], u32 (&ring)[D][8],
                                           const u8 *src, u64 B, u32 pa, u32 pb, u32 valid)
{
    (one_block<K, M, R0, NR, D, NT, Js>(acc, ring, src, B, pa, pb, valid), ...);
}

#ifndef SEC_FUSED_LDS_RING
#define SEC_FUSED_LDS_RING 8
#endif

template <int D, int W = 4>
struct LdsRing {
    u32x4 v[W][D][2][64];
};

template <int N>
__device__ __forceinline__ void wait_vm()
{
    asm volatile("s_waitcnt vmcnt(%0)" ::"i"(N) : "memory");
}

template <int K>
using Phase1Lds = std::conditional_t<(K >= 32), LdsRing<SEC_FUSED_LDS_RING>, char>;

template <int K, int M, int R0, int NR, int D, bool NT>
__device__ __forceinline__ void bs_span(const u8 *__restrict__ in, u8 *__restrict__ par, const sec::EncDesc &d, u32 s)
{
    static_assert(D >= 1 && D <= K, "ring depth");
    const u32 B = d.B;
    const u32 lane = (threadIdx.x & 63) * 16;
    const u32 pa = min(s + lane, B - 16), pb = min(s + 1024 + lane, B - 16);
    const u8 *src = in + d.in_off;

    u32 acc[NR * 8];
    u32 ring[D][8];
#pragma unroll
    for (int j = 0; j < D; ++j)
        load_block<NT>(ring[j], src + (u64)j * B, pa, pb, d.valid, j == K - 1);
    all_blocks<K, M, R0, NR, D, NT>(std::make_integer_sequence<int, K>{}, acc, ring, src, B, pa, pb, d.valid);

    u8 *dst = par + d.par_off;
#pragma unroll
    for (int r = 0; r < NR; ++r) {
        u32 y[8];
#pragma unroll
        for (int i = 0; i < 8; ++i)
            y[i] = acc[r * 8 + i];
        transpose8(y);
        u8 *o = dst + (u64)(R0 + r) * d.par_stride;
        st16(o + pa, y[0], y[1], y[2], y[3]);
        st16(o + pb, y[4], y[5], y[6], y[7]);
    }
}

template <int K, int M, int R0, int NR, int D>
__global__ __launch_bounds__(256) void sec_encode_bs_kernel(const u8 *__restrict__ in, u8 *__restrict__ par,
                                                            const sec::EncDesc *__restrict__ descs,
                                                            const sec::Tile *__restrict__ tiles)
{
    const sec::Tile tl = tiles[blockIdx.x];
    const sec::EncDesc d = descs[tl.chunk];
    const u32 s = tl.t0 + (threadIdx.x >> 6) * kSpan;
    if (s >= d.B)
        return;
    bs_span<K, M, R0, NR, D, true>(in, par, d, s);
}


struct PairXchg {
    u32x4 v[2][2][8][64];
};

__device__ __forceinline__ void barrier_lds()
{
    asm volatile("s_waitcnt lgkmcnt(0)\n\ts_barrier" ::: "memory");
}

template <int K, int M, int G, int NR, int D, int I>
__device__ __forceinline__ void pair_step(u32 (&acc)[NR * 8], u32 (&ring)[D][8], PairXchg &xb, const u8 *src, u64 B,
                                          u32 pa, u32 pb, u32 valid)
{
    constexpr int J = 2 * I + G, O = 2 * I + 1 - G;
    const u32 l = threadIdx.x & 63;
    u32 x[8];
#pragma unroll
    for (int i = 0; i < 8; ++i)
        x[i] = ring[I % D][i];
    if constexpr (I + D < K / 2)
        load_block<true>(ring[I % D], src + (u64)(2 * (I + D) + G) * B, pa, pb, valid, 2 * (I + D) + G == K - 1);
    transpose8(x);
    u32x4(&mine)[8][64] = xb.v[I & 1][G];
    u32x4(&theirs)[8][64] = xb.v[I & 1][1 - G];
    u32 lo[16], hi[16];
    subsets(x[0], x[1], x[2], x[3], lo);
    subsets(x[4], x[5], x[6], x[7], hi);
    mine[0][l] = u32x4{lo[1], lo[2], lo[3], lo[4]};
    mine[1][l] = u32x4{lo[5], lo[6], lo[7], lo[8]};
    mine[2][l] = u32x4{lo[9], lo[10], lo[11], lo[12]};
    mine[3][l] = u32x4{lo[13], lo[14], lo[15], hi[1]};
    mine[4][l] = u32x4{hi[2], hi[3], hi[4], hi[5]};
    mine[5][l] = u32x4{hi[6], hi[7], hi[8], hi[9]};
    mine[6][l] = u32x4{hi[10], hi[11], hi[12], hi[13]};
    mine[7][l] = u32x4{hi[14], hi[15], 0u, 0u};
    block_rows<K, M, G * NR, J, I == 0>(std::make_integer_sequence<int, NR * 8>{}, acc, lo, hi);
    barrier_lds();
    u32 lo2[16], hi2[16];
    const u32x4 t0 = theirs[0][l], t1 = theirs[1][l], t2 = theirs[2][l], t3 = theirs[3][l], t4 = theirs[4][l],
                t5 = theirs[5][l], t6 = theirs[6][l], t7 = theirs[7][l];
    lo2[0] = hi2[0] = 0;
    lo2[1] = t0.x, lo2[2] = t0.y, lo2[3] = t0.z, lo2[4] = t0.w;
    lo2[5] = t1.x, lo2[6] = t1.y, lo2[7] = t1.z, lo2[8] = t1.w;
    lo2[9] = t2.x, lo2[10] = t2.y, lo2[11] = t2.z, lo2[12] = t2.w;
    lo2[13] = t3.x, lo2[14] = t3.y, lo2[15] = t3.z, hi2[1] = t3.w;
    hi2[2] = t4.x, hi2[3] = t4.y, hi2[4] = t4.z, hi2[5] = t4.w;
    hi2[6] = t5.x, hi2[7] = t5.y, hi2[8] = t5.z, hi2[9] = t5.w;
    hi2[10] = t6.x, hi2[11] = t6.y, hi2[12] = t6.z, hi2[13] = t6.w;
    hi2[14] = t7.x, hi2[15] = t7.y;
    block_rows<K, M, G * NR, O, false>(std::make_integer_sequence<int, NR * 8>{}, acc, lo2, hi2);
}

template <int K, int M, int G, int NR, int D, int... Is>
__device__ __forceinline__ void pair_steps(std::integer_sequence<int, Is...>, u32 (&acc)[NR * 8], u32 (&ring)[D][8],
                                           PairXchg &xb, const u8 *src, u64 B, u32 pa, u32 pb, u32 valid)
{
    (pair_step<K, M, G, NR, D, Is>(acc, ring, xb, src, B, pa, pb, valid), ...);
}

template <int K, int M, int G, int NR, int D>
__device__ __forceinline__ void bs_pair_span(const u8 *__restrict__ in, u8 *__restrict__ par, const sec::EncDesc &d,
                                             u32 s, PairXchg &xb)
{
    static_assert(K % 2 == 0 && D >= 1 && D <= K / 2, "pair encode shape");
    const u32 B = d.B;
    const u32 lane = (threadIdx.x & 63) * 16;
    const u32 pa = min(s + lane, B - 16), pb = min(s + 1024 + lane, B - 16);
    const u8 *src = in + d.in_off;
    u32 ring[D][8];
#pragma unroll
    for (int j = 0; j < D; ++j)
        load_block<true>(ring[j], src + (u64)(2 * j + G) * B, pa, pb, d.valid, 2 * j + G == K - 1);
    u32 acc[NR * 8];
    pair_steps<K, M, G, NR, D>(std::make_integer_sequence<int, K / 2>{}, acc, ring, xb, src, B, pa, pb, d.valid);
    u8 *dst = par + d.par_off;
#pragma unroll
// ... 875 lines not shown
#endif
#ifndef SEC_FUSED_RING
#define SEC_FUSED_RING 6
#endif

struct BsShape {
    int k, m, nr, enc_ring, p1_ring;
    constexpr int groups() const { return (m - k + nr - 1) / nr; }
    constexpr int solve_nr() const { return k <= 16 ? k : 8; }
    constexpr int solve_ring() const { return SEC_SOLVE_RING < m - k ? SEC_SOLVE_RING : m - k; }
    constexpr int fused_nr() const { return k <= 10 ? k : 8; }
};
constexpr BsShape kShapes[] = {{10, 14, 4, 5, 5},  {8, 12, 4, 4, 4}, {16, 24, 8, 10, 10}, {32, 48, 16, 2, SEC_SYN_RING},
                               {64, 96, 16, SEC_BS_PAIR_RING, SEC_SYN_RING}, {8, 11, 3, 4, 4}};
constexpr int kNShapes = (int)(sizeof(kShapes) / sizeof(kShapes[0]));

template <class F, int... Is>
hipError_t dispatch_shape(int shape, F &&f, std::integer_sequence<int, Is...>)
{
    hipError_t e = hipErrorInvalidValue;
    ((shape == Is ? (void)(e = f(std::integral_constant<int, Is>{})) : void()), ...);
    return e;
}
template <class F>
hipError_t dispatch_shape(int shape, F &&f)
{
    return dispatch_shape(shape, f, std::make_integer_sequence<int, kNShapes>{});
}

template <class... P>
hipError_t launch(void (*kern)(P...), u32 nt, int lanes, size_t lds, void *stream, std::common_type_t<P>... args)
{
    void *a = nullptr, *b = nullptr;
    sec_next_launch_events(&a, &b);
    hipExtLaunchKernelGGL(kern, dim3(nt), dim3(lanes), lds, (hipStream_t)stream, (hipEvent_t)a, (hipEvent_t)b, 0,
                          args...);
    return hipGetLastError();
}

bool lanes_ok(int lanes) { return lanes >= 64 && lanes <= 256 && lanes % 64 == 0; }

}

int sec_bs_shape(int k, int m, int rows)
{
    for (int i = 0; i < kNShapes; ++i)
        if (kShapes[i].k == k && kShapes[i].m == m && (rows == 0 || kShapes[i].nr == rows))
            return i;
    return -1;
}

int sec_bs_groups(int shape) { return kShapes[shape].groups(); }

int sec_bs_rows(int shape) { return kShapes[shape].nr; }

uint32_t sec_bs_span() { return kSpan; }

int sec_solve_rows(int shape) { return shape >= 0 && shape < kNShapes ? kShapes[shape].solve_nr() : 0; }

int sec_solve_lds(int shape) { return shape == 3 || shape == 4; }

int sec_syn_pair(int shape) { return shape == 4; }

int sec_syn_shape(int k, int m) { return sec_bs_shape(k, m); }

int sec_launch_encode_bs(int shape, int group, int lanes, const uint8_t *in, uint8_t *par, const sec::EncDesc *descs,
                         const sec::Tile *t, uint32_t ntiles, void *stream)
{
    if (ntiles == 0)
        return hipSuccess;
    if (!lanes_ok(lanes) || (group != 0 && group != -2))
        return hipErrorInvalidValue;
    return dispatch_shape(shape, [&](auto i) {
        constexpr BsShape S = kShapes[decltype(i)::value];
        if (group != (S.groups() == 2 ? -2 : 0))
            return hipErrorInvalidValue;
        if constexpr (S.groups() == 2)
            return launch(sec_encode_bs_pair_kernel<S.k, S.m, S.nr, S.enc_ring>, ntiles, 128, 0, stream, in, par, descs, t);
        else
            return launch(sec_encode_bs_kernel<S.k, S.m, 0, S.nr, S.enc_ring>, ntiles, lanes, 0, stream, in, par, descs, t);
    });
}

int sec_launch_syndrome_bs(int shape, int lanes, const uint8_t *blocks, uint8_t *out, uint8_t *syn,
                           const sec::SynDesc *descs, const sec::Tile *t, uint32_t ntiles, sec::SynSlots sl,
                           void *stream)
{
    if (ntiles == 0)
        return hipSuccess;
    if (!lanes_ok(lanes))
        return hipErrorInvalidValue;
    return dispatch_shape(shape, [&](auto i) {
        constexpr BsShape S = kShapes[decltype(i)::value];
        constexpr auto kern = sec_syndrome_bs_kernel<S.k, S.m, S.nr, S.p1_ring>;
        return launch(kern, ntiles, lanes, 0, stream, blocks, out, syn, descs, t, sl);
    });
}

int sec_launch_syndrome_bs_pair(int shape, const uint8_t *blocks, uint8_t *out, uint8_t *syn, const sec::SynDesc *descs,
                                const sec::Tile *t, uint32_t ntiles, sec::SynSlots sl, void *stream)
{
    if (ntiles == 0)
        return hipSuccess;
    return dispatch_shape(shape, [&](auto i) {
        constexpr BsShape S = kShapes[decltype(i)::value];
        if constexpr (S.groups() == 2)
            return launch(sec_syndrome_bs_pair_kernel<S.k, S.m, S.nr, S.p1_ring>, ntiles, 128, 0, stream, blocks, out,
                          syn, descs, t, sl);
        else
            return hipErrorInvalidValue;
    });
}

int sec_launch_solve_bs(int shape, int lanes, const uint8_t *syn, uint8_t *out, const sec::SolveDesc *descs,
                        const sec::Tile *t, uint32_t ntiles, const uint64_t *masks, void *stream)
{
    if (ntiles == 0)
        return hipSuccess;
    if (!lanes_ok(lanes))
        return hipErrorInvalidValue;
    return dispatch_shape(shape, [&](auto i) {
        constexpr BsShape S = kShapes[decltype(i)::value];
        return launch(sec_solve_bs_kernel<S.k, S.m, S.solve_nr(), S.solve_ring()>, ntiles, lanes, 0, stream, syn, out,
                      descs, t, masks);
    });
}

int sec_launch_solve_bs_lds(int shape, int slots, const uint8_t *syn, uint8_t *out, const sec::SolveDesc *descs,
                            const sec::Tile *t, uint32_t ntiles, const uint64_t *masks, void *stream)
{
    if (ntiles == 0)
        return hipSuccess;
    return dispatch_shape(shape, [&](auto i) {
        constexpr BsShape S = kShapes[decltype(i)::value];
        if constexpr (S.k >= 32)
            return slots < 1 || slots > S.m - S.k
                       ? hipErrorInvalidValue
                       : launch(sec_solve_bs_lds_kernel<S.k, S.m, S.solve_nr()>, ntiles, 64 * (S.k / S.solve_nr()),
                                (size_t)slots * 2048, stream, syn, out, descs, t, masks);
        else
            return hipErrorInvalidValue;
    });
}

int sec_launch_decode_bs(int shape, int lanes, const uint8_t *blocks, uint8_t *out, const sec::SynDesc *descs,
                         const sec::Tile *t, uint32_t ntiles, sec::SynSlots sl, void *stream)
{
    if (ntiles == 0)
        return hipSuccess;
    if (!lanes_ok(lanes))
        return hipErrorInvalidValue;
    return dispatch_shape(shape, [&](auto i) {
        constexpr BsShape S = kShapes[decltype(i)::value];
        constexpr auto kern = sec_decode_bs_kernel<S.k, S.m, S.nr, S.fused_nr(), SEC_FUSED_RING>;
        return launch(kern, ntiles, lanes, 0, stream, blocks, out, descs, t, sl);
    });
}

int sec_launch_check_bs(int shape, int lanes, const uint8_t *blocks, uint8_t *out, const sec::CbsDesc *descs,
                        const sec::Tile *t, uint32_t ntiles, sec::CbsSlots sl, void *stream)
{
    if (ntiles == 0)
        return hipSuccess;
    if (!lanes_ok(lanes))
        return hipErrorInvalidValue;
    return dispatch_shape(shape, [&](auto i) {
// ... 20 lines not shown
```

storb_amd/engine.py:

```python

from __future__ import annotations

import contextlib
import ctypes
import os
import threading
import weakref

import numpy as np

from . import _lib
from ._lib import (CHK_DTYPE, CHK_RESULT_DTYPE, COPY_DTYPE, DCHK_DTYPE, DEC_DTYPE, ENC_DTYPE, MSG_DTYPE, RCHK_DTYPE,
                   REP_DTYPE, SEC_F_ASYNC, SEC_F_GPU_PARITY_IDS, SEC_F_HOST, SEC_F_RECOVER, SEC_F_STAGED)


class Error(Exception):
    """A zfec precondition violation (zfec raises ``zfec.Error`` for the same cases)."""


class ECRuntimeError(RuntimeError):
    """Device / runtime failure (no GPU, HIP error, out of memory)."""


def check(rc: int, lib=None) -> None:
# ... 317 lines not shown
        for it in items:
            check_repair_check_item(*it)
        if not items:
            return ([], [], []) if digests else ([], [])
        sn, bo, _keep, slot0 = self._lay_out_blocks(items)
        tn, to, dig, objs, tgt0, _views = self._lay_out_targets(items, digests)
        descs = np.zeros(len(items), dtype=RCHK_DTYPE)
        for j, (k, m, blocks, _sharenums, targets) in enumerate(items):
            descs[j] = (len(blocks[0]), slot0[j], tgt0[j], len(targets), len(blocks), k, m)
        res, rb, col = self._result_arrays(len(items), sn.size)
        self.repair_check_batch(descs, sn, bo, 0, tn, to, 0, res, digests=dig, row_bad=rb, column=col, host=True)
        out, digs = self._targets_done(objs, dig)
        checks = self._check_results(items, slot0, res, rb, col)
        return (out, digs, checks) if digests else (out, checks)

    def encode_digest_batch(self, descs: np.ndarray, src, parity, digests, *, host: bool = False,
                            asynchronous: bool = False) -> None:
        descs = np.ascontiguousarray(descs, dtype=ENC_DTYPE)
        s, _ks = addr(src)
        p, _kp = addr(parity)
        g, _kg = addr(digests)
        flags = (SEC_F_HOST if host else 0) | (SEC_F_ASYNC if asynchronous else 0)
        self._check(self.lib.sec_encode_digest_batch(self._ctx, _ptr(descs), len(descs), s or None, p or None,
                                                     g or None, flags))

    @staticmethod
    def _key_handle(key):
        h = getattr(key, "handle", key)
        if not h:
            raise ECRuntimeError("tagged encode needs an open ModKey")
        return h

    def encode_tag_batch(self, descs: np.ndarray, src, parity, tags, key, *, digests=None, host: bool = False,
                         asynchronous: bool = False) -> None:
        descs = np.ascontiguousarray(descs, dtype=ENC_DTYPE)
        s, _ks = addr(src)
        p, _kp = addr(parity)
        t, _kt = addr(tags)
        g, _kg = addr(digests) if digests is not None else (0, None)
        flags = (SEC_F_HOST if host else 0) | (SEC_F_ASYNC if asynchronous else 0)
        self._check(self.lib.sec_encode_tag_batch(self._ctx, self._key_handle(key), _ptr(descs), len(descs),
                                                  s or None, p or None, g or None, t or None, flags))

    @staticmethod
    def _tag_ints(tags: np.ndarray, ms) -> list[list[int]]:
        tv = memoryview(tags)
        out, f = [], 0
        for m in ms:
            out.append([int.from_bytes(tv[256 * (f + j):256 * (f + j + 1)], "big") for j in range(m)])
            f += m
        return out

    def sha1_batch(self, msgs: np.ndarray, digests, *, host: bool = False, asynchronous: bool = False) -> None:
        msgs = np.ascontiguousarray(msgs, dtype=MSG_DTYPE)
        g, _kg = addr(digests)
        flags = (SEC_F_HOST if host else 0) | (SEC_F_ASYNC if asynchronous else 0)
        self._check(self.lib.sec_sha1_batch(self._ctx, _ptr(msgs), len(msgs), g or None, flags))

    def host_empty(self, nbytes: int) -> np.ndarray:
        n = int(nbytes)
        p = ctypes.c_void_p()
        self._check(self.lib.sec_host_alloc(self._ctx, max(n, 1), ctypes.byref(p)))
        raw = (ctypes.c_uint8 * max(n, 1)).from_address(p.value)
        weakref.finalize(raw, self.lib.sec_host_free, None, p.value).atexit = False
        return np.frombuffer(raw, dtype=np.uint8, count=n)

    def register(self, buf) -> None:
        a, keep = addr(buf)
        self._check(self.lib.sec_host_register(self._ctx, a, keep.nbytes if keep is not None else len(buf)))

    def unregister(self, buf) -> None:
        a, _ = addr(buf)
        self._check(self.lib.sec_host_unregister(None, a))

    def host_paths(self) -> tuple[int, int, int]:
        z, r, st = ctypes.c_int64(0), ctypes.c_int64(0), ctypes.c_int64(0)
        self._check(self.lib.sec_ctx_host_paths(self._ctx, ctypes.byref(z), ctypes.byref(r), ctypes.byref(st)))
        return z.value, r.value, st.value

    def decode_paths(self) -> tuple[int, int]:
        syn, direct = ctypes.c_int64(0), ctypes.c_int64(0)
        self._check(self.lib.sec_ctx_decode_paths(self._ctx, ctypes.byref(syn), ctypes.byref(direct)))
        return syn.value, direct.value

    def decode_methods(self) -> tuple[int, int, int, int]:
        f, p, t, d = (ctypes.c_int64(0) for _ in range(4))
        self._check(self.lib.sec_ctx_decode_methods(self._ctx, ctypes.byref(f), ctypes.byref(p), ctypes.byref(t),
                                                    ctypes.byref(d)))
        return f.value, p.value, t.value, d.value

    def check_methods(self) -> tuple[int, int]:
        b, d = ctypes.c_int64(0), ctypes.c_int64(0)
        self._check(self.lib.sec_ctx_check_methods(self._ctx, ctypes.byref(b), ctypes.byref(d)))
        return b.value, d.value

    def repair_methods(self) -> tuple[int, int]:
        b, d = ctypes.c_int64(0), ctypes.c_int64(0)
        self._check(self.lib.sec_ctx_repair_methods(self._ctx, ctypes.byref(b), ctypes.byref(d)))
        return b.value, d.value

    _SCRATCH_CAP = 256 << 20

    def _out_buffer(self, nbytes: int) -> np.ndarray:
        n = max(int(nbytes), 1)
        if n > self._SCRATCH_CAP:
            return np.empty(n, dtype=np.uint8)
        cur = getattr(self, "_scratch", None)
        if cur is None or cur.size < n:
            cur = self._scratch = self.host_empty(max(n, 2 * (cur.size if cur is not None else 0), 1 << 20))
        return cur[:n]

    def sha1_host(self, datas) -> list[bytes]:
        msgs = np.zeros(len(datas), dtype=MSG_DTYPE)
        keep = []
        for i, d in enumerate(datas):
            a, kp = addr(d)
            keep.append(kp)
            ln = len(kp) if isinstance(kp, np.ndarray) else len(d)
            msgs[i] = (a, ln, ln)
        out = np.empty(max(20 * len(datas), 1), dtype=np.uint8)
        self.sha1_batch(msgs, out, host=True)
        mv = memoryview(out)
        return [bytes(mv[20 * i:20 * (i + 1)]) for i in range(len(datas))]

    def encode_host_raw(self, chunks, shapes, digests: bool = False, staged: bool = False, tag_key=None):
        n = len(chunks)
        descs = np.zeros(n, dtype=ENC_DTYPE)
        keep = []
        layout = []
        total = 0
        for i, (c, (k, m)) in enumerate(zip(chunks, shapes)):
            a, kp = addr(c)
            keep.append(kp)
            ln = len(kp) if isinstance(kp, np.ndarray) else len(c)
            B = -(-ln // k) if ln else 0
            descs[i] = (a, ln, total, max(B, 1), k, m)
            layout.append((total, B, m - k))
            total += (m - k) * B
        out = self._out_buffer(total)
        if tag_key is not None:
            ms = [m for (_, m) in shapes]
            dig = np.empty(max(20 * sum(ms), 1), dtype=np.uint8) if digests else None
            tags = np.empty(max(256 * sum(ms), 1), dtype=np.uint8)
            if n:
                self.encode_tag_batch(descs, 0, out, tags, tag_key, digests=dig, host=True)
            ints = self._tag_ints(tags, ms)
            return (out, layout, dig, ints) if digests else (out, layout, ints)
        if digests:
            dig = np.empty(max(20 * sum(m for (_, m) in shapes), 1), dtype=np.uint8)
            if n:
                self.encode_digest_batch(descs, 0, out, dig, host=True)
            return out, layout, dig
        if n:
            self.encode_batch(descs, 0, out, host=True, staged=staged)
        return out, layout

    def encode_pieces_into(self, chunks, shapes, piece_addrs, digests: np.ndarray | None = None,
                           staged: bool = False, gpu_parity_ids: bool = False, tags: np.ndarray | None = None,
                           tag_key=None) -> None:
        n = len(chunks)
        descs = np.zeros(n, dtype=ENC_DTYPE)
        keep = []
        for i, (c, (k, m)) in enumerate(zip(chunks, shapes)):
            a, kp = addr(c)
            keep.append(kp)
            ln = len(kp) if isinstance(kp, np.ndarray) else len(c)
# ... 508 lines not shown
```

Measured before the change: 3353 GiB/s.

## Derive encode tiles and descriptors affinely on device instead of uploading per-chunk records

Adds an affine plan that spots runs of uniformly strided chunks and launches kernels that compute each block's tile and descriptor from blockIdx with magic-number division, instead of reading per-tile records from an uploaded metadata image. It skips building and copying descriptor and tile arrays when every tile is covered, and cuts per-block global loads. By default it applies only to non-wide encode bins at 64 lanes; decode support is present but off unless the mode is forced. It adds integer math per block and more planning work on the host.

```diff
diff --git a/include/storb_ec.h b/include/storb_ec.h
--- a/include/storb_ec.h
+++ b/include/storb_ec.h
@@ -240,6 +240,8 @@
 int sec_ctx_host_paths(sec_ctx *ctx, int64_t *zero_copy, int64_t *registered, int64_t *staged);
 int sec_host_pinned_bytes(int64_t *loaned, int64_t *idle);
 int sec_ctx_decode_paths(sec_ctx *ctx, int64_t *syndrome, int64_t *direct);
+int sec_ctx_set_affine(sec_ctx *ctx, int mode);
+int sec_ctx_affine_launches(sec_ctx *ctx, int64_t *affine, int64_t *record);
 int sec_ctx_decode_methods(sec_ctx *ctx, int64_t *fused, int64_t *pair, int64_t *two_kernel, int64_t *direct);
 int sec_memcpy(sec_ctx *ctx, void *dst, const void *src, size_t bytes, int kind);
 int sec_memset(sec_ctx *ctx, void *dptr, int value, size_t bytes);
diff --git a/storb_amd/_build.py b/storb_amd/_build.py
--- a/storb_amd/_build.py
+++ b/storb_amd/_build.py
@@ -13,7 +13,7 @@
 VARIANT_DIR = os.path.join(ROOT, "build", "variants")
 INCLUDE = os.path.join(ROOT, "include")
 SOURCES = ["kernels.hip", "kernels_bs.hip", "bignum.hip", "api.cpp"]
-HEADERS = ["kernels.hpp", "bignum.hpp", "bn_host.hpp", "bs_plan.hpp", "gf_host.hpp", "gf_const.hpp",
+HEADERS = ["affine_plan.hpp", "kernels.hpp", "bignum.hpp", "bn_host.hpp", "bs_plan.hpp", "gf_host.hpp", "gf_const.hpp",
            "task_pool.hpp"]
 ARCH = "gfx950"
 HIPCC = os.environ.get("HIPCC", "/opt/rocm/bin/hipcc")
diff --git a/storb_amd/_lib.py b/storb_amd/_lib.py
--- a/storb_amd/_lib.py
+++ b/storb_amd/_lib.py
@@ -172,6 +172,8 @@
                                           ctypes.POINTER(ctypes.c_int64)]),
     "sec_host_pinned_bytes": (ctypes.c_int, [ctypes.POINTER(ctypes.c_int64), ctypes.POINTER(ctypes.c_int64)]),
     "sec_ctx_decode_paths": (ctypes.c_int, [_vp, ctypes.POINTER(ctypes.c_int64), ctypes.POINTER(ctypes.c_int64)]),
+    "sec_ctx_set_affine": (ctypes.c_int, [_vp, ctypes.c_int]),
+    "sec_ctx_affine_launches": (ctypes.c_int, [_vp, ctypes.POINTER(ctypes.c_int64), ctypes.POINTER(ctypes.c_int64)]),
     "sec_ctx_decode_methods": (ctypes.c_int, [_vp, ctypes.POINTER(ctypes.c_int64), ctypes.POINTER(ctypes.c_int64),
                                               ctypes.POINTER(ctypes.c_int64), ctypes.POINTER(ctypes.c_int64)]),
     "sec_memcpy": (ctypes.c_int, [_vp, _vp, _vp, ctypes.c_size_t, ctypes.c_int]),
diff --git a/storb_amd/csrc/affine_plan.hpp b/storb_amd/csrc/affine_plan.hpp
--- /dev/null
+++ b/storb_amd/csrc/affine_plan.hpp
@@ -0,0 +1,156 @@
+#pragma once
+#include <stdint.h>
+
+#include <algorithm>
+#include <vector>
+
+#include "kernels.hpp"
+
+#if defined(__HIPCC__)
+#define SEC_HD __host__ __device__
+#else
+#define SEC_HD
+#endif
+
+namespace sec {
+
+inline uint32_t affine_magic(uint32_t d) { return (uint32_t)std::min<uint64_t>(0xFFFFFFFFull, (1ull << 32) / d); }
+
+SEC_HD inline uint32_t affine_div(uint32_t b, uint32_t d, uint32_t magic, uint32_t &rem)
+{
+    uint32_t q = (uint32_t)(((uint64_t)b * magic) >> 32);
+    uint32_t r = b - q * d;
+    if (r >= d) {
+        ++q;
+        r -= d;
+    }
+    rem = r;
+    return q;
+}
+
+struct TileMap {
+    uint32_t tpc, tpc_magic;
+    uint32_t tpg, tpg_magic;
+    uint32_t step;
+    uint32_t r0;
+    uint32_t rstep;
+    uint32_t ntail;
+};
+
+SEC_HD inline Tile affine_tile(const TileMap &m, uint32_t b)
+{
+    uint32_t rem, i;
+    const uint32_t c = affine_div(b, m.tpc, m.tpc_magic, rem);
+    const uint32_t g = affine_div(rem, m.tpg, m.tpg_magic, i);
+    return Tile{c, i * m.step, m.r0 + g * m.rstep, i + 1 == m.tpg ? m.ntail : 0u};
+}
+
+inline bool affine_map_of(const Tile *t, uint32_t n, TileMap &m)
+{
+    if (n == 0)
+        return false;
+    uint32_t tpg = 1;
+    while (tpg < n && t[tpg].r0 == t[0].r0)
+        ++tpg;
+    if (n % tpg)
+        return false;
+    m.tpc = n;
+    m.tpc_magic = affine_magic(n);
+    m.tpg = tpg;
+    m.tpg_magic = affine_magic(tpg);
+    m.step = tpg > 1 ? t[1].t0 - t[0].t0 : 0;
+    m.r0 = t[0].r0;
+    m.rstep = n > tpg ? t[tpg].r0 - t[0].r0 : 0;
+    m.ntail = t[tpg - 1].ntail;
+    for (uint32_t b = 0; b < n; ++b) {
+        const Tile a = affine_tile(m, b);
+        if (a.chunk != 0 || a.t0 != t[b].t0 || a.r0 != t[b].r0 || a.ntail != t[b].ntail)
+            return false;
+    }
+    return true;
+}
+
+struct EncAffine {
+    EncDesc d0;
+    uint64_t in_step, par_step;
+    TileMap map;
+};
+
+SEC_HD inline EncDesc affine_desc(const EncAffine &a, uint32_t c)
+{
+    EncDesc d = a.d0;
+    d.in_off += (uint64_t)c * a.in_step;
+    d.par_off += (uint64_t)c * a.par_step;
+    return d;
+}
+
+struct DecAffine {
+    DecDesc d0;
+    uint64_t out_step;
+    uint64_t off[kBatchVecs], off_step[kBatchVecs];
+    uint32_t row[kBatchVecs], miss[kBatchVecs], avail[kBatchVecs];
+    TileMap map;
+};
+
+struct AffineClass {
+    int nshape = 0, naddr = 0;
+    std::vector<uint64_t> id;
+    std::vector<uint64_t> tiles;
+    std::vector<uint64_t> shape;
+    std::vector<uint64_t> addr;
+    size_t size() const { return id.size(); }
+    void add(uint64_t chunk, uint64_t ntiles, const uint64_t *sh, const uint64_t *ad)
+    {
+        id.push_back(chunk);
+        tiles.push_back(ntiles);
+        shape.insert(shape.end(), sh, sh + nshape);
+        addr.insert(addr.end(), ad, ad + naddr);
+    }
+};
+
+struct AffineRun {
+    size_t first = 0, count = 0;
+    uint64_t tiles = 0;
+};
+
+inline AffineRun affine_find(const AffineClass &c)
+{
+    const size_t n = c.size();
+    AffineRun best;
+    if (n == 0)
+        return best;
+    auto same_shape = [&](size_t a, size_t b) {
+        return c.id[b] == c.id[a] + (b - a) && c.tiles[a] == c.tiles[b] &&
+               std::equal(c.shape.begin() + a * c.nshape, c.shape.begin() + (a + 1) * c.nshape,
+                          c.shape.begin() + b * c.nshape);
+    };
+    auto same_step = [&](size_t j) {
+        const uint64_t *p = &c.addr[0] + (j - 2) * c.naddr, *q = p + c.naddr, *r = q + c.naddr;
+        for (int f = 0; f < c.naddr; ++f)
+            if (r[f] - q[f] != q[f] - p[f])
+                return false;
+        return true;
+    };
+    uint64_t total = 0;
+    for (size_t i = 0; i < n; ++i)
+        total += c.tiles[i];
+    auto close = [&](size_t s, size_t e) {
+        const uint64_t t = (uint64_t)(e - s) * c.tiles[s];
+        if (t > best.tiles || best.count == 0)
+            best = AffineRun{s, e - s, t};
+    };
+    size_t s = 0;
+    for (size_t j = 1; j < n; ++j) {
+        const bool shape_ok = same_shape(j - 1, j);
+        if (shape_ok && (j - s < 2 || c.naddr == 0 || same_step(j)))
+            continue;
+        close(s, j);
+        s = shape_ok ? j - 1 : j;
+    }
+    close(s, n);
+    if (best.tiles * 2 < total)
+        return AffineRun{};
+    return best;
+}
+
+}
diff --git a/storb_amd/csrc/api.cpp b/storb_amd/csrc/api.cpp
--- a/storb_amd/csrc/api.cpp
+++ b/storb_amd/csrc/api.cpp
@@ -16,6 +16,7 @@
 #include <vector>
 
 #include "task_pool.hpp"
+#include "affine_plan.hpp"
 #include "bignum.hpp"
 #include "bn_host.hpp"
 #include "bs_plan.hpp"
@@ -243,11 +244,17 @@
     uint32_t first, count;
     int mfma = 0;
 };
+struct AffineGroup {
+    Group g;
+    sec::EncAffine enc;
+    sec::DecAffine dec;
+};
 using KeyedLaunches = std::vector<std::pair<int, std::pair<uint32_t, uint32_t>>>;
 
 struct SubPlan {
     int64_t c0 = 0, c1 = 0;
     std::vector<Group> groups;
+    std::vector<AffineGroup> affine;
     size_t off_desc = 0, off_tiles = 0, off_tail = 0, off_soff = 0, off_srow = 0, off_mrow = 0, off_savail = 0;
     uint32_t ntail = 0;
     uint64_t in_bytes = 0, out_bytes = 0;
@@ -496,6 +503,126 @@
     return tiles;
 }
 
+bool affine_rule(int mode, bool decode, int kind, int lanes)
+{
+    if (mode >= 0)
+        return mode == 1;
+    return !decode && kind == 0 && lanes == 64;
+}
+
+template <class Desc, class Fields>
+sec::AffineClass affine_class(const std::vector<sec::Tile> &tiles, const std::vector<Desc> &descs, int nshape, int naddr,
+                              Fields fields, std::vector<size_t> &start)
+{
+    sec::AffineClass cls;
+    cls.nshape = nshape;
+    cls.naddr = naddr;
+    std::vector<uint64_t> sh((size_t)nshape), ad((size_t)naddr);
+    for (size_t i = 0; i < tiles.size();) {
+        size_t j = i + 1;
+        while (j < tiles.size() && tiles[j].chunk == tiles[i].chunk)
+            ++j;
+        fields(descs[tiles[i].chunk], sh.data(), ad.data());
+        cls.add(tiles[i].chunk, j - i, sh.data(), ad.data());
+        start.push_back(i);
+        i = j;
+    }
+    start.push_back(tiles.size());
+    return cls;
+}
+
+void take_affine_encode(int mode, const std::vector<sec::EncDesc> &descs, Bins &bins, std::vector<AffineGroup> &out)
+{
+    if (mode == 0 || SEC_XCD_ORDER == 1)
+        return;
+    for (auto &kv : bins) {
+        const auto [kind, rows, U, lanes, wide] = kv.first;
+        std::vector<sec::Tile> &tiles = kv.second;
+        const bool bs = kind == 3;
+        if (tiles.empty() || wide || (bs ? U != 0 : (kind != 0 || U != 1)) || !affine_rule(mode, false, kind, lanes))
+            continue;
+        std::vector<size_t> start;
+        const sec::AffineClass cls = affine_class(
+            tiles, descs, 6, 2,
+            [](const sec::EncDesc &d, uint64_t *sh, uint64_t *ad) {
+                const uint64_t f[6] = {d.B, d.k, d.p, d.tab, d.valid, d.par_stride};
+                std::copy(f, f + 6, sh);
+                ad[0] = d.in_off;
+                ad[1] = d.par_off;
+            },
+            start);
+        const sec::AffineRun run = sec::affine_find(cls);
+        if (run.count == 0 || run.tiles > 0xFFFFFFFFull)
+            continue;
+        AffineGroup ag{};
+        const size_t t0 = start[run.first], t1 = start[run.first + run.count];
+        if (!sec::affine_map_of(&tiles[t0], (uint32_t)cls.tiles[run.first], ag.enc.map))
+            continue;
+        const sec::EncDesc &d0 = descs[cls.id[run.first]];
+        ag.enc.d0 = d0;
+        ag.enc.in_step = run.count > 1 ? descs[cls.id[run.first] + 1].in_off - d0.in_off : 0;
+        ag.enc.par_step = run.count > 1 ? descs[cls.id[run.first] + 1].par_off - d0.par_off : 0;
+        ag.g = Group{rows, U, lanes, wide, 0, (uint32_t)(t1 - t0), kind};
+        tiles.erase(tiles.begin() + t0, tiles.begin() + t1);
+        out.push_back(ag);
+    }
+}
+
+void take_affine_decode(int mode, const std::vector<sec::DecDesc> &descs, const std::vector<uint64_t> &soff,
+                        const std::vector<uint32_t> &srow, const std::vector<uint32_t> &mrow,
+                        const std::vector<uint32_t> &savail, Bins &bins, std::vector<AffineGroup> &out)
+{
+    if (mode == 0 || SEC_XCD_ORDER == 1)
+        return;
+    constexpr int KS = sec::kBatchVecs;
+    for (auto &kv : bins) {
+        const auto [kind, rows, U, lanes, wide] = kv.first;
+        std::vector<sec::Tile> &tiles = kv.second;
+        if (tiles.empty() || wide || U != 1 || !affine_rule(mode, true, kind, lanes))
+            continue;
+        std::vector<size_t> start;
+        const sec::AffineClass cls = affine_class(
+            tiles, descs, 6 + 3 * KS, 1 + KS,
+            [&](const sec::DecDesc &d, uint64_t *sh, uint64_t *ad) {
+                const uint64_t f[6] = {d.B, d.k, d.e, d.tab, d.valid, d.n};
+                std::copy(f, f + 6, sh);
+                std::fill(sh + 6, sh + 6 + 3 * KS, 0);
+                std::fill(ad, ad + 1 + KS, 0);
+                ad[0] = d.out_off;
+                for (uint32_t c = 0; c < d.k; ++c) {
+                    sh[6 + c] = srow[d.slot0 + c];
+                    sh[6 + KS + c] = mrow[d.slot0 + c];
+                    sh[6 + 2 * KS + c] = savail[d.slot0 + c];
+                    ad[1 + c] = soff[d.slot0 + c];
+                }
+            },
+            start);
+        const sec::AffineRun run = sec::affine_find(cls);
+        if (run.count == 0 || run.tiles > 0xFFFFFFFFull)
+            continue;
+        AffineGroup ag{};
+        const size_t t0 = start[run.first], t1 = start[run.first + run.count];
+        if (!sec::affine_map_of(&tiles[t0], (uint32_t)cls.tiles[run.first], ag.dec.map))
+            continue;
+        const sec::DecDesc &d0 = descs[cls.id[run.first]];
+        const sec::DecDesc *d1 = run.count > 1 ? &descs[cls.id[run.first] + 1] : nullptr;
+        sec::DecAffine &a = ag.dec;
+        a.d0 = d0;
+        a.d0.slot0 = 0;
+        a.out_step = d1 ? d1->out_off - d0.out_off : 0;
+        for (uint32_t c = 0; c < d0.k; ++c) {
+            a.off[c] = soff[d0.slot0 + c];
+            a.off_step[c] = d1 ? soff[d1->slot0 + c] - soff[d0.slot0 + c] : 0;
+            a.row[c] = srow[d0.slot0 + c];
+            a.miss[c] = mrow[d0.slot0 + c];
+            a.avail[c] = savail[d0.slot0 + c];
+        }
+        ag.g = Group{rows, U, lanes, wide, 0, (uint32_t)(t1 - t0), kind};
+        tiles.erase(tiles.begin() + t0, tiles.begin() + t1);
+        out.push_back(ag);
+    }
+}
+
 template <class InBytes>
 std::vector<std::pair<int64_t, int64_t>> slab_ranges(bool host, int64_t nchunks, InBytes in_bytes, size_t slab)
 {
@@ -576,6 +703,8 @@
     int64_t syn_chunks = 0, direct_chunks = 0, fused_chunks = 0;
     int64_t chk_bs_chunks = 0, chk_direct_chunks = 0;
     int64_t rep_bs_chunks = 0, rep_direct_chunks = 0;
+    int affine_mode = -1;
+    int64_t affine_launches = 0, record_launches = 0;
 
     hipStream_t stream() const { return ext ? ext : own; }
     hipEvent_t ev()
@@ -743,12 +872,14 @@
     for (const auto &pe : pending)
         coef_off.push_back(img.put(pe.coef.data(), pe.coef.size()));
     const size_t bytes = img.bytes.size();
-    RC(pin_wait(ctx));
-    RC(ctx->pin.ensure(bytes));
-    memcpy(ctx->pin.p, img.bytes.data(), bytes);
-    RC(plan.meta.ensure(bytes));
-    CK(hipMemcpyAsync(plan.meta.p, ctx->pin.p, bytes, hipMemcpyHostToDevice, ctx->stream()));
-    CK(hipEventRecord(ctx->pin_ev, ctx->stream()));
+    if (bytes) {
+        RC(pin_wait(ctx));
+        RC(ctx->pin.ensure(bytes));
+        memcpy(ctx->pin.p, img.bytes.data(), bytes);
+        RC(plan.meta.ensure(bytes));
+        CK(hipMemcpyAsync(plan.meta.p, ctx->pin.p, bytes, hipMemcpyHostToDevice, ctx->stream()));
+        CK(hipEventRecord(ctx->pin_ev, ctx->stream()));
+    }
     for (size_t i = 0; i < pending.size(); ++i) {
         int e = sec_launch_expand(plan.meta.as<uint8_t>(coef_off[i]), (uint32_t)pending[i].coef.size(),
                                   tc.buf.as<uint32_t>() + pending[i].dst, ctx->stream());
@@ -1010,9 +1141,12 @@
             else if (p > 0)
                 add_work(bins, tail, (uint32_t)(i - c0), B, valid, p, c.k, false, narrow);
         }
+        take_affine_encode(ctx->affine_mode, descs, bins, sp.affine);
         std::vector<sec::Tile> tiles;
         flatten(bins, sp.groups, tiles, false);
         sp.ntail = (uint32_t)tail.size();
+        if (tiles.empty() && tail.empty())
+            descs.clear();
         sp.dig_off = sp.out_bytes;
         if (host && digest)
             sp.out_bytes += (uint64_t)msgs.size() * 20;
@@ -1044,6 +1178,15 @@
     const sec::EncDesc *dd = plan.meta.as<sec::EncDesc>(sp.off_desc);
     const sec::Tile *dt = plan.meta.as<sec::Tile>(sp.off_tiles);
     const uint32_t *tabs = ctx->enc_tabs.buf.as<uint32_t>();
+    for (const AffineGroup &ag : sp.affine) {
+        const Group &g = ag.g;
+        int e = g.mfma == 3 ? sec_launch_encode_bs_affine(g.rows, g.lanes, in, par, ag.enc, g.count, s)
+                            : sec_launch_encode_affine(g.rows, g.lanes, in, par, ag.enc, g.count, tabs, s);
+        if (e)
+            return hip_fail((hipError_t)e, g.mfma == 3 ? "sec_encode_bs_affine_kernel" : "sec_encode_affine_kernel");
+    }
+    ctx->affine_launches += (int64_t)sp.affine.size();
+    ctx->record_launches += (int64_t)sp.groups.size();
     for (const Group &g : sp.groups) {
         int e = g.mfma == 3 ? sec_launch_encode_bs(g.rows, g.U == kBsPair ? -2 : g.U, g.lanes, in, par, dd,
                                                    dt + g.first, g.count, s)
@@ -1395,8 +1538,16 @@
                 if (kv.first >= kSolveLds && big(kv.second, vB))
                     xcd_order(kv.second);
         }
+        take_affine_decode(ctx->affine_mode, descs, soff, srow, mrow, savail, bins, sp.affine);
         std::vector<sec::Tile> tiles;
         flatten(bins, sp.groups, tiles, true);
+        if (tiles.empty() && tail.empty()) {
+            descs.clear();
+            soff.clear();
+            srow.clear();
+            mrow.clear();
+            savail.clear();
+        }
         const std::vector<sec::Tile> stl = flatten_keyed(stiles, sp.syn1), vtl = flatten_keyed(vtiles, sp.syn2),
                                      ftl = flatten_keyed(ftiles, sp.synf);
         sp.off_ftiles = img.put(ftl.data(), ftl.size() * sizeof(sec::Tile));
@@ -1411,7 +1562,8 @@
         sp.off_desc = img.put(descs.data(), descs.size() * sizeof(sec::DecDesc));
         sp.off_tiles = img.put(tiles.data(), tiles.size() * sizeof(sec::Tile));
         sp.off_tail = img.put(tail.data(), tail.size() * sizeof(sec::TailItem));
-        soff.resize(soff.size() + sec::kBatchVecs, 0);
+        if (!soff.empty())
+            soff.resize(soff.size() + sec::kBatchVecs, 0);
         sp.off_soff = img.put(soff.data(), soff.size() * 8);
         sp.off_srow = img.put(srow.data(), srow.size() * 4);
         sp.off_mrow = img.put(mrow.data(), mrow.size() * 4);
@@ -1431,6 +1583,13 @@
     const uint32_t *tabs = ctx->dec_tabs.buf.as<uint32_t>();
     const sec::DecSlots sl{plan.meta.as<uint64_t>(sp.off_soff), plan.meta.as<uint32_t>(sp.off_srow),
                            plan.meta.as<uint32_t>(sp.off_mrow), plan.meta.as<uint32_t>(sp.off_savail)};
+    for (const AffineGroup &ag : sp.affine) {
+        int e = sec_launch_decode_affine(ag.g.rows, ag.g.lanes, ag.g.mfma, blocks, out, ag.dec, ag.g.count, tabs, s);
+        if (e)
+            return hip_fail((hipError_t)e, "sec_decode_affine_kernel");
+    }
+    ctx->affine_launches += (int64_t)sp.affine.size();
+    ctx->record_launches += (int64_t)sp.groups.size();
     for (const Group &g : sp.groups) {
         int e = sec_launch_rows(g.rows, g.U, g.wide, g.lanes, blocks, out, dd, dt + g.first, g.count, tabs, sl, s,
                                 g.mfma);
@@ -3922,6 +4081,28 @@
     return SEC_OK;
 }
 
+int sec_ctx_set_affine(sec_ctx *ctx, int mode)
+{
+    if (!ctx || mode < -1 || mode > 1)
+        return SEC_EINVAL;
+    if (ctx->affine_mode == mode)
+        return SEC_OK;
+    RC(set_dev(ctx));
+    RC(drain_all(ctx));
+    ctx->affine_mode = mode;
+    ctx->enc_plan.valid = ctx->dec_plan.valid = false;
+    return SEC_OK;
+}
+
+int sec_ctx_affine_launches(sec_ctx *ctx, int64_t *affine, int64_t *record)
+{
+    if (!ctx || !affine || !record)
+        return SEC_EINVAL;
+    *affine = ctx->affine_launches;
+    *record = ctx->record_launches;
+    return SEC_OK;
+}
+
 int sec_ctx_decode_methods(sec_ctx *ctx, int64_t *fused, int64_t *pair, int64_t *two_kernel, int64_t *direct)
 {
     if (!ctx)
diff --git a/storb_amd/csrc/kernels.hip b/storb_amd/csrc/kernels.hip
--- a/storb_amd/csrc/kernels.hip
+++ b/storb_amd/csrc/kernels.hip
@@ -3,6 +3,7 @@
 
 #include <type_traits>
 
+#include "affine_plan.hpp"
 #include "kernels.hpp"
 
 using u8 = uint8_t;
@@ -303,6 +304,21 @@
         encode_ragged<R>(in, par, d, tl, tabs);
 }
 
+template <int R>
+__global__ __launch_bounds__(sec::max_lanes(R, 1)) void sec_encode_affine_kernel(const u8 *__restrict__ in,
+                                                                                 u8 *__restrict__ par,
+                                                                                 const sec::EncAffine a,
+                                                                                 const u32 *__restrict__ tabs)
+{
+    const sec::Tile tl = sec::affine_tile(a.map, blockIdx.x);
+    const sec::EncDesc d = sec::affine_desc(a, tl.chunk);
+    const u32 t = tl.t0 + threadIdx.x * sec::kLaneBytes;
+    if (t < d.valid)
+        encode_main<R, 1, false>(in, par, d, tl, tabs, t);
+    if (tl.ntail)
+        encode_ragged<R>(in, par, d, tl, tabs);
+}
+
 template <int R, int U, bool W>
 __device__ __forceinline__ void encode_main(const u8 *__restrict__ in, u8 *__restrict__ par, const sec::EncDesc &d,
                                             const sec::Tile &tl, const u32 *__restrict__ tabs, u32 t)
@@ -434,14 +450,14 @@
     }
 }
 
-template <int R, int U, bool W, int KBX>
+template <int R, int U, bool W, int KBX, class Slots>
 __device__ __forceinline__ void decode_main(const u8 *__restrict__ blocks, u8 *__restrict__ out,
                                             const sec::DecDesc &d, const sec::Tile &tl, u32 t,
-                                            const u32 *__restrict__ tabs, const sec::DecSlots sl);
-template <int R>
+                                            const u32 *__restrict__ tabs, const Slots sl);
+template <int R, class Slots>
 __device__ __forceinline__ void decode_ragged(const u8 *__restrict__ blocks, u8 *__restrict__ out, const sec::DecDesc &d,
                                            const sec::Tile &tl, const u32 *__restrict__ tabs,
-                                           const sec::DecSlots sl);
+                                           const Slots sl);
 
 template <int R, int U, bool W, int KBX>
 __global__ __launch_bounds__(sec::max_lanes(R, U)) void sec_decode_kernel(const u8 *__restrict__ blocks, u8 *__restrict__ out,
@@ -459,10 +475,38 @@
         decode_ragged<R>(blocks, out, d, tl, tabs, sl);
 }
 
-template <int R>
+struct AffineOff {
+    const u64 *base, *step;
+    u32 chunk, i0;
+    __device__ __forceinline__ AffineOff operator+(u32 n) const { return AffineOff{base, step, chunk, i0 + n}; }
+    __device__ __forceinline__ u64 operator[](u32 i) const { return base[i0 + i] + (u64)chunk * step[i0 + i]; }
+};
+struct DecAffineSlots {
+    AffineOff off;
+    const u32 *row, *miss, *avail;
+};
+
+template <int R, int KBX>
+__global__ __launch_bounds__(sec::max_lanes(R, 1)) void sec_decode_affine_kernel(const u8 *__restrict__ blocks,
+                                                                                 u8 *__restrict__ out,
+                                                                                 const sec::DecAffine a,
+                                                                                 const u32 *__restrict__ tabs)
+{
+    const sec::Tile tl = sec::affine_tile(a.map, blockIdx.x);
+    sec::DecDesc d = a.d0;
+    d.out_off += (u64)tl.chunk * a.out_step;
+    const DecAffineSlots sl{AffineOff{a.off, a.off_step, tl.chunk, 0}, a.row, a.miss, a.avail};
+    const u32 t = tl.t0 + threadIdx.x * sec::kLaneBytes;
+    if (t < d.valid)
+        decode_main<R, 1, false, KBX>(blocks, out, d, tl, t, tabs, sl);
+    if (tl.ntail)
+        decode_ragged<R>(blocks, out, d, tl, tabs, sl);
+}
+
+template <int R, class Slots>
 __device__ __forceinline__ void decode_ragged(const u8 *__restrict__ blocks, u8 *__restrict__ out, const sec::DecDesc &d,
                                               const sec::Tile &tl, const u32 *__restrict__ tabs,
-                                              const sec::DecSlots sl)
+                                              const Slots sl)
 {
     for (u32 i = ragged_lane0(d.valid, tl.t0); i < tl.ntail; i += blockDim.x) {
         const u32 tp = d.valid + i;
@@ -493,11 +537,11 @@
     }
 }
 
-template <int R, int U, bool W, int KBX>
+template <int R, int U, bool W, int KBX, class Slots>
 __device__ __forceinline__ void decode_main(const u8 *__restrict__ blocks, u8 *__restrict__ out,
                                             const sec::DecDesc &d, const sec::Tile &tl, u32 t,
                                             const u32 *__restrict__ tabs,
-                                                         const sec::DecSlots sl)
+                                                         const Slots sl)
 {
     const u32 B = d.B, k = d.k;
     u32 pos[U];
@@ -519,7 +563,7 @@
         constexpr bool LT = lds_tab<R, true>();
         const u32x2 *vt = wave_tabs<KB, R, LT>(tj, tstep, c0, k);
         u64 so[KB];
-        const u64 *sop = sl.off + d.slot0 + c0;
+        const auto sop = sl.off + d.slot0 + c0;
 #pragma unroll
         for (int c = 0; c < KB; ++c)
             so[c] = sop[c];
@@ -1820,6 +1864,41 @@
     return dispatch_enc<1, false>(rows, in, par, descs, tiles, ntiles, tabs, (u32)lanes, s);
 }
 
+int sec_launch_encode_affine(int rows, int lanes, const uint8_t *in, uint8_t *par, const sec::EncAffine &a,
+                             uint32_t ntiles, const uint32_t *tabs, void *stream)
+{
+    if (ntiles == 0)
+        return hipSuccess;
+    if (lanes < 64 || lanes % 64 || lanes > sec::max_lanes(rows, 1) || a.d0.k > (uint32_t)sec::kBatchVecs)
+        return hipErrorInvalidValue;
+    return with_rows<1>(rows, [&](auto r) {
+        constexpr int R = decltype(r)::value;
+        return launch_shm(sec_encode_affine_kernel<R>, dim3(ntiles), dim3((u32)lanes),
+                          lds_tab_bytes<batch_blocks<1, false, false>(), R, false>((u32)lanes), (hipStream_t)stream, in,
+                          par, a, tabs);
+    });
+}
+
+int sec_launch_decode_affine(int rows, int lanes, int kb, const uint8_t *blocks, uint8_t *out, const sec::DecAffine &a,
+                             uint32_t ntiles, const uint32_t *tabs, void *stream)
+{
+    if (ntiles == 0)
+        return hipSuccess;
+    if (lanes < 64 || lanes % 64 || lanes > sec::max_lanes(rows, 1) || (kb != 0 && kb != 4) ||
+        a.d0.k > (uint32_t)(kb ? kb : sec::kBatchVecs))
+        return hipErrorInvalidValue;
+    return with_rows<0>(rows, [&](auto r) {
+        constexpr int R = decltype(r)::value;
+        auto go = [&](auto kbx) {
+            constexpr int KBX = decltype(kbx)::value;
+            constexpr int KB = KBX > 0 ? KBX : batch_blocks<1, false, true>();
+            return launch_shm(sec_decode_affine_kernel<R, KBX>, dim3(ntiles), dim3((u32)lanes),
+                              lds_tab_bytes<KB, R, true>((u32)lanes), (hipStream_t)stream, blocks, out, a, tabs);
+        };
+        return kb ? go(std::integral_constant<int, 4>{}) : go(std::integral_constant<int, 0>{});
+    });
+}
+
 int sec_launch_encode_tail(const uint8_t *in, uint8_t *par, const sec::EncDesc *descs, const sec::TailItem *items,
                            uint32_t nitems, const uint32_t *tabs, void *stream)
 {
diff --git a/storb_amd/csrc/kernels.hpp b/storb_amd/csrc/kernels.hpp
--- a/storb_amd/csrc/kernels.hpp
+++ b/storb_amd/csrc/kernels.hpp
@@ -254,6 +254,13 @@
                         const sec::Tile *t, uint32_t ntiles, const uint64_t *masks, void *stream);
 int sec_launch_encode_tail(const uint8_t *in, uint8_t *par, const sec::EncDesc *descs, const sec::TailItem *items,
                            uint32_t nitems, const uint32_t *tabs, void *stream);
+namespace sec { struct EncAffine; struct DecAffine; }
+int sec_launch_decode_affine(int rows, int lanes, int kb, const uint8_t *blocks, uint8_t *out, const sec::DecAffine &a,
+                             uint32_t ntiles, const uint32_t *tabs, void *stream);
+int sec_launch_encode_affine(int rows, int lanes, const uint8_t *in, uint8_t *par, const sec::EncAffine &a,
+                             uint32_t ntiles, const uint32_t *tabs, void *stream);
+int sec_launch_encode_bs_affine(int shape, int lanes, const uint8_t *in, uint8_t *par, const sec::EncAffine &a,
+                                uint32_t ntiles, void *stream);
 int sec_launch_sha1(const uint8_t *base0, const uint8_t *base1, const sec::MsgDesc *msgs, uint32_t nmsgs,
                     uint8_t *digests, void *stream, int split = 0);
 template <class Desc, class Slots>
diff --git a/storb_amd/csrc/kernels_bs.hip b/storb_amd/csrc/kernels_bs.hip
--- a/storb_amd/csrc/kernels_bs.hip
+++ b/storb_amd/csrc/kernels_bs.hip
@@ -8,6 +8,7 @@
 #include <utility>
 
 #include "gf_const.hpp"
+#include "affine_plan.hpp"
 #include "kernels.hpp"
 
 namespace {
@@ -247,6 +248,18 @@
 {
     const sec::Tile tl = tiles[blockIdx.x];
     const sec::EncDesc d = descs[tl.chunk];
+    const u32 s = tl.t0 + (threadIdx.x >> 6) * kSpan;
+    if (s >= d.B)
+        return;
+    bs_span<K, M, R0, NR, D, true>(in, par, d, s);
+}
+
+template <int K, int M, int R0, int NR, int D>
+__global__ __launch_bounds__(256) void sec_encode_bs_affine_kernel(const u8 *__restrict__ in, u8 *__restrict__ par,
+                                                                   const sec::EncAffine a)
+{
+    const sec::Tile tl = sec::affine_tile(a.map, blockIdx.x);
+    const sec::EncDesc d = sec::affine_desc(a, tl.chunk);
     const u32 s = tl.t0 + (threadIdx.x >> 6) * kSpan;
     if (s >= d.B)
         return;
@@ -1288,6 +1301,22 @@
     });
 }
 
+int sec_launch_encode_bs_affine(int shape, int lanes, const uint8_t *in, uint8_t *par, const sec::EncAffine &a,
+                                uint32_t ntiles, void *stream)
+{
+    if (ntiles == 0)
+        return hipSuccess;
+    if (!lanes_ok(lanes))
+        return hipErrorInvalidValue;
+    return dispatch_shape(shape, [&](auto i) {
+        constexpr BsShape S = kShapes[decltype(i)::value];
+        if constexpr (S.groups() == 2)
+            return hipErrorInvalidValue;
+        else
+            return launch(sec_encode_bs_affine_kernel<S.k, S.m, 0, S.nr, S.enc_ring>, ntiles, lanes, 0, stream, in, par, a);
+    });
+}
+
 int sec_launch_syndrome_bs(int shape, int lanes, const uint8_t *blocks, uint8_t *out, uint8_t *syn,
                            const sec::SynDesc *descs, const sec::Tile *t, uint32_t ntiles, sec::SynSlots sl,
                            void *stream)
diff --git a/storb_amd/engine.py b/storb_amd/engine.py
--- a/storb_amd/engine.py
+++ b/storb_amd/engine.py
@@ -423,6 +423,14 @@
         syn, direct = ctypes.c_int64(0), ctypes.c_int64(0)
         self._check(self.lib.sec_ctx_decode_paths(self._ctx, ctypes.byref(syn), ctypes.byref(direct)))
         return syn.value, direct.value
+
+    def set_affine(self, mode: int) -> None:
+        self._check(self.lib.sec_ctx_set_affine(self._ctx, int(mode)))
+
+    def affine_launches(self) -> tuple[int, int]:
+        a, r = ctypes.c_int64(0), ctypes.c_int64(0)
+        self._check(self.lib.sec_ctx_affine_launches(self._ctx, ctypes.byref(a), ctypes.byref(r)))
+        return a.value, r.value
 
     def decode_methods(self) -> tuple[int, int, int, int]:
         f, p, t, d = (ctypes.c_int64(0) for _ in range(4))
```

Result: no change. 3438 GiB/s, median of 4 (+2.5%).
